# LPMP/BDD

Hardware: AMD Instinct MI355X
Metric: parallel-MMA iterations/sec, 10.5M BDD nodes, 1 GPU (+ achieved HBM GB/s in roofline) (higher is better)
Workload: dtype f32

## Files before the change

bdd_amd/capi.py:

```python
from __future__ import annotations

import ctypes as C
import os
import subprocess

_HERE = os.path.dirname(os.path.abspath(__file__))
LIB_PATH = os.path.abspath(os.environ["BDDMMA_LIB"]) if os.environ.get("BDDMMA_LIB") else os.path.join(_HERE, "csrc", "libbdd_mma_hip.so")

OK = 0
ERR_INVALID_ARGUMENT, ERR_INVALID_BDD, ERR_DEVICE, ERR_STATE, ERR_UNSUPPORTED, ERR_IO = -1, -2, -3, -4, -5, -6
F32, F64 = 0, 1
K_FORWARD_MM, K_BACKWARD_MM, K_FINISH_DELTA, K_OTHER, K_COUNT = 0, 1, 2, 3, 4


class Options(C.Structure):
    _fields_ = [("pack_width", C.c_uint32), ("wide_pack_width", C.c_uint32), ("deterministic", C.c_uint32),
                ("vars_per_bin", C.c_uint32), ("stage_cap", C.c_uint32), ("waves_per_block", C.c_uint32),
                ("keep_bdd_order", C.c_uint32), ("resident_sweeps", C.c_uint32), ("exchange_by_variable", C.c_uint32),
                ("variant_flags", C.c_uint32), ("pack_fill", C.c_uint32), ("pack_stagger", C.c_uint32)]


class LbfgsParams(C.Structure):
    _fields_ = [("history_size", C.c_int32), ("init_step_size", C.c_double), ("req_rel_lb_increase", C.c_double),
                ("step_size_decrease_factor", C.c_double), ("step_size_increase_factor", C.c_double)]


class LbfgsState(C.Structure):
    _fields_ = [("step_size", C.c_double), ("last_applied_step", C.c_double), ("mma_iterations", C.c_uint64),
                ("lbfgs_iterations", C.c_uint64), ("history_entries", C.c_int32), ("num_unsuccessful_updates", C.c_int32),
                ("last_kind", C.c_int32), ("last_trials", C.c_int32)]


class RunResult(C.Structure):
    _fields_ = [("iterations", C.c_uint64), ("lb_initial", C.c_double), ("lb_final", C.c_double),
                ("seconds", C.c_double), ("stop_reason", C.c_int32)]


class Profile(C.Structure):
    _fields_ = [("launches", C.c_uint64 * K_COUNT), ("total_ms", C.c_double * K_COUNT)]


_V, _U64, _I, _D = C.c_void_p, C.c_uint64, C.c_int, C.c_double
SIGNATURES = {
    "bddmma_create": (_I, [C.POINTER(_V), _I, _I, _V, _V, _U64, _V, _U64, C.POINTER(Options)]),
    "bddmma_destroy": (None, [_V]),
    "bddmma_device_count": (_I, []),
    "bddmma_device_chip": (_I, [_I, C.POINTER(C.c_uint32), C.POINTER(C.c_uint32), C.POINTER(C.c_uint64)]),
    "bddmma_set_layout_threads": (_I, [_I]),
    "bddmma_set_thread_layout_threads": (_I, [_I]),
    "bddmma_last_error": (C.c_char_p, [_V]),
    "bddmma_nr_variables": (_U64, [_V]),
    "bddmma_nr_bdds": (_U64, [_V]),
    "bddmma_nr_layers": (_U64, [_V]),
    "bddmma_nr_bdd_nodes": (_U64, [_V]),
    "bddmma_nr_hops": (_U64, [_V]),
    "bddmma_nr_packs": (_U64, [_V]),
    "bddmma_solve_sweep_kind": (_I, [_V]),
    "bddmma_fused_small": (_I, [_V]),
    "bddmma_fused_small_learned": (_I, [_V]),
    "bddmma_nontemporal_loads": (_I, [_V]),
    "bddmma_precision": (_I, [_V]),
    "bddmma_device": (_I, [_V]),
    "bddmma_num_bdds_per_var": (_I, [_V, _V]),
    "bddmma_layer_variables": (_I, [_V, _V]),
    "bddmma_layer_bdds": (_I, [_V, _V]),
    "bddmma_nodes_per_hop": (_I, [_V, _V]),
    "bddmma_layers_per_hop": (_I, [_V, _V]),
    "bddmma_update_costs": (_I, [_V, _V, _U64, _V, _U64, _I, _I]),
    "bddmma_set_cost": (_I, [_V, _D, _U64]),
    "bddmma_get_solver_costs": (_I, [_V, _V, _V, _V, _I]),
    "bddmma_set_solver_costs": (_I, [_V, _V, _V, _V, _I]),
    "bddmma_primal_objective_vec": (_I, [_V, _V, _I]),
    "bddmma_forward_run": (_I, [_V]),
    "bddmma_backward_run": (_I, [_V]),
    "bddmma_lower_bound": (_I, [_V, C.POINTER(_D)]),
    "bddmma_lower_bound_per_bdd": (_I, [_V, _V, _I]),
    "bddmma_iteration": (_I, [_V, _D]),
    "bddmma_iterations": (_I, [_V, _D, _U64]),
    "bddmma_learned_iterations": (_I, [_V, _V, _I, _U64, _D, _D, _V, _V, _V, _U64, _D, _I, C.POINTER(_U64)]),
    "bddmma_learned_iterations_omega_vec": (_I, [_V, _V, _I, _U64, _V, _I, _D, _V, _V, _V, _U64, _D, _I, C.POINTER(_U64)]),
    "bddmma_isotropic_dist_weights": (_I, [_V, _V, _I]),
    "bddmma_forward_mm": (_I, [_V, _D, _V, _I]),
    "bddmma_backward_mm": (_I, [_V, _D, _V, _I]),
    "bddmma_normalize_delta": (_I, [_V, _V, _I]),
    "bddmma_distribute_delta": (_I, [_V]),
    "bddmma_get_delta": (_I, [_V, _V, _I]),
    "bddmma_set_delta": (_I, [_V, _V, _I]),
    "bddmma_min_marginals": (_I, [_V, _I, _V, _V, _V, _I]),
    "bddmma_min_marginal_diff": (_I, [_V, _V, _I]),
    "bddmma_sum_marginals": (_I, [_V, _I, _I, _V, _V, _V, _I]),
    "bddmma_smooth_solution": (_I, [_V, _V, _I]),
    "bddmma_grad_min_marginal_diff": (_I, [_V, _V, _V, _V, _I]),
    "bddmma_grad_lower_bound_per_bdd": (_I, [_V, _V, _V, _V, _I, _I]),
    "bddmma_grad_distribute_delta": (_I, [_V, _V, _V, _V, _I]),
    "bddmma_grad_cost_perturbation": (_I, [_V, _V, _V, _V, _V, _I]),
    "bddmma_grad_learned_iterations": (_I, [_V, _V, _I, _D, _V, _I, _V, _V, _V, _V, _V, _U64, _U64, _U64, _I]),
    "bddmma_bdds_solution": (_I, [_V, _I, _V, _I]),
    "bddmma_net_solver_costs": (_I, [_V, _V, _I]),
    "bddmma_make_dual_feasible": (_I, [_V, _V, _I]),
    "bddmma_gradient_step": (_I, [_V, _V, _D, _I]),
    "bddmma_lbfgs_create": (_I, [C.POINTER(_V), _V, C.POINTER(LbfgsParams)]),
    "bddmma_lbfgs_destroy": (None, [_V]),
    "bddmma_lbfgs_iteration": (_I, [_V]),
    "bddmma_lbfgs_update_costs": (_I, [_V, _V, _U64, _V, _U64, _I, _I]),
    "bddmma_lbfgs_flush": (_I, [_V]),
    "bddmma_lbfgs_get_state": (_I, [_V, C.POINTER(LbfgsState)]),
    "bddmma_perturb_primal_costs": (_I, [_V, _V, _D, C.c_uint32, C.c_uint32, C.POINTER(C.c_uint32), _V, _V, _V]),
    "bddmma_run_solver": (_I, [_V, _V, _U64, _D, _D, _D, _I, C.POINTER(RunResult)]),
    "bddmma_run_solver_host_loop": (_I, [_V, _V, _U64, _D, _D, _D, _I, C.POINTER(RunResult)]),
    "bddmma_batch_create": (_I, [C.POINTER(_V), C.POINTER(_V), _U64]),
    "bddmma_batch_destroy": (None, [_V]),
    "bddmma_batch_last_error": (C.c_char_p, [_V]),
    "bddmma_batch_size": (_U64, [_V]),
    "bddmma_batch_iterations": (_I, [_V, _D, _U64]),
    "bddmma_learned_iterations_batch": (_I, [_V, _V, _V, _D, _U64, _I]),
    "bddmma_grad_learned_iterations_batch": (_I, [_V, _V, _V, _D, _V, _V, _V, _V, _V, _U64, _U64, _U64, _I]),
    "bddmma_set_solver_costs_batch": (_I, [_V, _V, _V, _V, _I]),
    "bddmma_get_solver_costs_batch": (_I, [_V, _V, _V, _V, _I]),
    "bddmma_stream_wait_batch": (_I, [_V, _V]),
    "bddmma_stream_signal_batch": (_I, [_V, _V]),
    "bddmma_batch_time_iterations": (_I, [_V, _D, _U64, C.POINTER(_D)]),
    "bddmma_batch_run_solver": (_I, [_V, _U64, _D, _D, _D, C.POINTER(RunResult)]),
    "bddmma_batch_lower_bounds": (_I, [_V, C.POINTER(_D)]),
    "bddmma_incremental_mm_agreement_rounding": (_I, [_V, _V, _D, _D, _U64, _U64, C.c_uint32, _I, _V, C.POINTER(_I)]),
    "bddmma_save": (_I, [_V, C.c_char_p]),
    "bddmma_load": (_I, [C.POINTER(_V), _I, C.c_char_p]),
    "bddmma_synchronize": (_I, [_V]),
    "bddmma_stream_wait": (_I, [_V, _V]),
    "bddmma_stream_signal": (_I, [_V, _V]),
    "bddmma_set_profiling": (_I, [_V, _I]),
    "bddmma_get_profile": (_I, [_V, C.POINTER(Profile)]),
    "bddmma_time_iterations": (_I, [_V, _D, _U64, C.POINTER(_D)]),
    "bddmma_time_kernel": (_I, [_V, _I, _U64, C.POINTER(_D)]),
    "bddmma_device_bytes": (_U64, [_V]),
    "bddmma_device_allocated_bytes": (_U64, [_V]),
    "bddmma_layout_create": (_I, [C.POINTER(_V), _V, _V, _U64, C.POINTER(Options)]),
    "bddmma_layout_create_for_chip": (_I, [C.POINTER(_V), _V, _V, _U64, C.POINTER(Options), _I, C.c_uint32, C.c_uint32]),
    "bddmma_layout_destroy": (None, [_V]),
    "bddmma_layout_size": (_U64, [_V, _I]),
    "bddmma_layout_copy": (_I, [_V, _I, _V]),
    "bddmma_layout_res2_records": (_I, [_V, _I, _V, _V, _V]),
    "bddmma_layout_stream_records": (_I, [_V, _I, _V, _V, _V]),
    "bddmma_layout_layer_records": (_I, [_V, _I, _V, _V, _V]),
# ... 68 lines not shown
```

bdd_amd/csrc/capi.cpp:

```cpp
#include <chrono>
#include <cmath>
#include <cstdio>
#include <cstdlib>
#include <cstring>
#include <limits>
#include <new>
#include <string>
#include <vector>

#include "../../include/bdd_mma.h"
#include "layout.hpp"
#include "solver.hpp"

using namespace bddmma;

struct bddmma_lbfgs;
extern "C" int bddmma_lbfgs_iteration(bddmma_lbfgs* l);
extern "C" int bddmma_lbfgs_update_costs(bddmma_lbfgs* l, const void* lo, uint64_t n_lo, const void* hi, uint64_t n_hi, int elem_precision,
                                         int on_device);

namespace {
thread_local std::string g_err;

template <typename F>
// ... 49 lines not shown
        constexpr bool timing = false;
#endif
        auto t_last = std::chrono::steady_clock::now();
        auto lap = [&](const char* what) {
            if (!timing) return;
            const auto now = std::chrono::steady_clock::now();
            std::fprintf(stderr, "[create] %-28s %8.1f ms\n", what, std::chrono::duration<double, std::milli>(now - t_last).count());
            t_last = now;
        };
        HostLayout L;
        ChipInfo chip;
        int rc = query_chip(device, &chip, g_err);
        if (rc) return rc;
        rc = build_layout(instr, bdd_delims, n_bdds, opts, L, g_err, false, precision == BDDMMA_F64 ? 8 : 4, chip);
        if (rc) return rc;
        lap("host layout");
        SolverBase* impl = nullptr;
        rc = create_solver(&impl, precision, device, L, opts, g_err);
        if (rc) return rc;
        lap("device buffers + upload");
        impl->n_packs_narrow = L.narrow.n_packs();
        impl->n_packs_wide = L.wide.n_packs() + L.huge.n_packs();
        if (costs_hi && n_costs) {
            rc = impl->update_costs(nullptr, 0, costs_hi, n_costs, BDDMMA_F64, 0);
            if (rc) {
                g_err = impl->err;
                delete impl;
                return rc;
            }
        }
        lap("update_costs");
        *out = new bddmma_solver{impl};
        return BDDMMA_OK;
    } catch (const std::exception& e) {
        g_err = e.what();
        return BDDMMA_ERR_DEVICE;
    }
}

int bddmma_device_count(void) { return device_count(); }
int bddmma_device_chip(int device, uint32_t* n_cus, uint32_t* lds_bytes_per_cu, uint64_t* max_resident_threads)
{
    if (device < 0 || device >= device_count()) { g_err = "no such HIP device"; return BDDMMA_ERR_DEVICE; }
    ChipInfo chip;
    const int rc = query_chip(device, &chip, g_err);
    if (rc) return rc;
    if (n_cus) *n_cus = chip.n_cus;
    if (lds_bytes_per_cu) *lds_bytes_per_cu = chip.lds_bytes;
    if (max_resident_threads) *max_resident_threads = chip.max_resident_threads;
    return BDDMMA_OK;
}
int bddmma_set_layout_threads(int n)
{
    if (n < 0) return BDDMMA_ERR_INVALID_ARGUMENT;
    set_layout_threads((unsigned)n);
    return BDDMMA_OK;
}
int bddmma_set_thread_layout_threads(int n)
{
    if (n < 0) return BDDMMA_ERR_INVALID_ARGUMENT;
    set_thread_layout_threads((unsigned)n);
    return BDDMMA_OK;
}

void bddmma_destroy(bddmma_solver* s)
{
    if (!s) return;
    delete s->impl;
    delete s;
}

const char* bddmma_last_error(const bddmma_solver* s) { return (s && s->impl) ? s->impl->err.c_str() : g_err.c_str(); }

uint64_t bddmma_nr_variables(const bddmma_solver* s) { return s && s->impl ? s->impl->n_vars : 0; }
uint64_t bddmma_nr_bdds(const bddmma_solver* s) { return s && s->impl ? s->impl->n_bdds : 0; }
uint64_t bddmma_nr_layers(const bddmma_solver* s) { return s && s->impl ? s->impl->n_layers : 0; }
uint64_t bddmma_nr_bdd_nodes(const bddmma_solver* s) { return s && s->impl ? s->impl->n_input_nodes : 0; }
uint64_t bddmma_nr_hops(const bddmma_solver* s) { return s && s->impl ? s->impl->n_hops : 0; }
uint64_t bddmma_nr_packs(const bddmma_solver* s) { return s && s->impl ? s->impl->n_packs_narrow + s->impl->n_packs_wide : 0; }
int bddmma_solve_sweep_kind(const bddmma_solver* s) { return s && s->impl ? s->impl->solve_sweep_kind : -1; }
int bddmma_fused_small(const bddmma_solver* s) { return s && s->impl ? (s->impl->fused_small ? 1 : 0) : -1; }
int bddmma_fused_small_learned(const bddmma_solver* s) { return s && s->impl ? (s->impl->fused_small_learned ? 1 : 0) : -1; }
int bddmma_nontemporal_loads(const bddmma_solver* s) { return s && s->impl ? (s->impl->nt_loads ? 1 : 0) : -1; }
int bddmma_precision(const bddmma_solver* s) { return s && s->impl ? s->impl->precision : -1; }
int bddmma_device(const bddmma_solver* s) { return s && s->impl ? s->impl->device : -1; }
uint64_t bddmma_device_bytes(const bddmma_solver* s) { return s && s->impl ? s->impl->dev_bytes : 0; }
uint64_t bddmma_device_allocated_bytes(const bddmma_solver* s) { return s && s->impl ? s->impl->dev_alloc_bytes : 0; }

int bddmma_num_bdds_per_var(const bddmma_solver* s, int32_t* out)
{
    return guarded(s, [&](SolverBase* b) { return copy_host(b->h_nbdds, out); });
}
int bddmma_layer_variables(const bddmma_solver* s, int32_t* out)
{
    return guarded(s, [&](SolverBase* b) { return copy_host(b->h_layer_var, out); });
}
int bddmma_layer_bdds(const bddmma_solver* s, int32_t* out)
{
    return guarded(s, [&](SolverBase* b) { return copy_host(b->h_layer_bdd, out); });
}
int bddmma_nodes_per_hop(const bddmma_solver* s, uint64_t* out)
{
    return guarded(s, [&](SolverBase* b) { return copy_host(b->nodes_per_hop, out); });
}
int bddmma_layers_per_hop(const bddmma_solver* s, uint64_t* out)
{
    return guarded(s, [&](SolverBase* b) { return copy_host(b->layers_per_hop, out); });
}

int bddmma_update_costs(bddmma_solver* s, const void* lo, uint64_t n_lo, const void* hi, uint64_t n_hi,
                        int elem_precision, int on_device)
{
    return guarded(s, [&](SolverBase* b) {
        if (elem_precision != BDDMMA_F32 && elem_precision != BDDMMA_F64) {
            b->err = "elem_precision must be BDDMMA_F32 or BDDMMA_F64";
            return BDDMMA_ERR_INVALID_ARGUMENT;
        }
        return b->update_costs(lo, n_lo, hi, n_hi, elem_precision, on_device);
    });
}
int bddmma_set_cost(bddmma_solver* s, double c, uint64_t var)
{
    return guarded(s, [&](SolverBase* b) { return b->set_cost(c, var); });
}
int bddmma_get_solver_costs(const bddmma_solver* s, void* lo, void* hi, void* mm, int on_device)
{
    return guarded(s, [&](SolverBase* b) { return b->get_solver_costs(lo, hi, mm, on_device); });
}
int bddmma_set_solver_costs(bddmma_solver* s, const void* lo, const void* hi, const void* mm, int on_device)
{
    return guarded(s, [&](SolverBase* b) { return b->set_solver_costs(lo, hi, mm, on_device); });
}
int bddmma_primal_objective_vec(bddmma_solver* s, void* out, int on_device)
{
    return guarded(s, [&](SolverBase* b) { return b->primal_objective_vec(out, on_device); });
}
int bddmma_forward_run(bddmma_solver* s) { return guarded(s, [&](SolverBase* b) { return b->forward_run(); }); }
int bddmma_backward_run(bddmma_solver* s) { return guarded(s, [&](SolverBase* b) { return b->backward_run(); }); }
int bddmma_lower_bound(bddmma_solver* s, double* lb)
{
    return guarded(s, [&](SolverBase* b) { return lb ? b->lower_bound(lb) : BDDMMA_ERR_INVALID_ARGUMENT; });
}
int bddmma_lower_bound_per_bdd(bddmma_solver* s, void* out, int on_device)
{
    return guarded(s, [&](SolverBase* b) { return b->lower_bound_per_bdd(out, on_device); });
}
int bddmma_iteration(bddmma_solver* s, double omega)
{
    return guarded(s, [&](SolverBase* b) { return b->iteration(omega); });
}
int bddmma_iterations(bddmma_solver* s, double omega, uint64_t n)
{
    return guarded(s, [&](SolverBase* b) { return b->iterations(omega, n); });
}
int bddmma_learned_iterations(bddmma_solver* s, const void* dist_weights, int weights_on_device, uint64_t num_itr, double omega,
                              double improvement_slope, void* sol_avg, void* lb_first_diff_avg, void* lb_second_diff_avg,
                              uint64_t compute_history_for_itr, double history_avg_beta, int outputs_on_device, uint64_t* itr_done)
{
    return guarded(s, [&](SolverBase* b) {
        return b->learned_iterations(dist_weights, weights_on_device, num_itr, omega, improvement_slope, sol_avg, lb_first_diff_avg,
                                     lb_second_diff_avg, compute_history_for_itr, history_avg_beta, outputs_on_device, itr_done, nullptr, 0);
    });
}
int bddmma_learned_iterations_omega_vec(bddmma_solver* s, const void* dist_weights, int weights_on_device, uint64_t num_itr, const void* omega_vec,
                                        int omega_vec_on_device, double improvement_slope, void* sol_avg, void* lb_first_diff_avg,
                                        void* lb_second_diff_avg, uint64_t compute_history_for_itr, double history_avg_beta, int outputs_on_device,
// ... 611 lines not shown
```

bdd_amd/csrc/kernels.hpp:

```cpp
#pragma once
#include <hip/hip_runtime.h>

#include <cstdint>
#include <type_traits>

#include "layout.hpp"

#include "kernels/common.hpp"
#include "kernels/stream.hpp"
#include "kernels/narrow.hpp"
#include "kernels/resident.hpp"
#include "kernels/narrow2.hpp"
#include "kernels/narrow3.hpp"
#include "kernels/wide.hpp"
#include "kernels/exchange.hpp"
#include "kernels/small.hpp"
#include "kernels/elementwise.hpp"
```

bdd_amd/csrc/solver.hpp:

```cpp
#pragma once
#include <hip/hip_runtime.h>

#include <cstdint>
#include <limits>
#include <memory>
#include <string>
#include <utility>
#include <vector>

#include "../../include/bdd_mma.h"
#include "layout.hpp"

namespace bddmma {

struct SolverBase {
    int precision = BDDMMA_F32, device = -1;
    hipStream_t stream = nullptr;
    std::string err;
    uint64_t n_vars = 0, n_bdds = 0, n_layers = 0, n_hops = 0, n_input_nodes = 0, n_slots = 0;
    int solve_sweep_kind = 0;
    uint32_t pack_width = 0, wide_pack_width = 0, wide_slot_base = 0;
    uint64_t dev_bytes = 0;
    uint64_t dev_alloc_bytes = 0;
    bool fwd_valid = false, bwd_valid = false;
    uint64_t cost_epoch = 0;
    bool deterministic = false;
    std::vector<uint64_t> nodes_per_hop, layers_per_hop;
    std::vector<int32_t> h_nbdds, h_layer_var, h_layer_bdd;
    std::vector<uint32_t> h_var_ptr;
    uint32_t n_packs_narrow = 0, n_packs_wide = 0;
    LayoutScalars lay_scalars{};
    bddmma_options saved_opts{};
    virtual int download_layout(HostLayout& H) = 0;
    virtual int init_from_layout(const HostLayout& L, const bddmma_options* opts) = 0;

    bool profiling = false;
    uint32_t prof_stride = 1;
    uint64_t prof_iter = 0;
    bool prof_active = false;
    std::vector<std::pair<hipEvent_t, hipEvent_t>> ev_pool;
    std::vector<int> ev_class;
    size_t ev_used = 0;
    hipEvent_t ev_t0 = nullptr, ev_t1 = nullptr;
    hipEvent_t ev_order = nullptr;

    virtual ~SolverBase() {}
    virtual int forward_run() = 0;
    virtual int backward_run() = 0;
    virtual int lower_bound(double* lb) = 0;
    virtual int lower_bound_enqueue(int slot) = 0;
    virtual int lower_bound_fetch(int slot, double* lb) = 0;
    virtual int lower_bound_per_bdd(void* out, int on_device) = 0;
    virtual int iteration(double omega) = 0;
    virtual int iterations(double omega, uint64_t n)
    {
        for (uint64_t i = 0; i < n; ++i)
            if (int rc = iteration(omega)) return rc;
        return BDDMMA_OK;
    }
    virtual int learned_iterations(const void* dist_weights, int weights_on_device, uint64_t num_itr, double omega, double improvement_slope,
                                   void* sol_avg, void* lb_first_diff_avg, void* lb_second_diff_avg, uint64_t compute_history_for_itr,
                                   double history_avg_beta, int outputs_on_device, uint64_t* itr_done, const void* omega_vec,
                                   int omega_vec_on_device) = 0;
    virtual int isotropic_dist_weights(void* out, int on_device) = 0;
    double initial_lb_change = std::numeric_limits<double>::infinity();
    std::shared_ptr<int> lbfgs_attached = std::make_shared<int>(0);
    bool fused_small = false;
    bool fused_small_learned = false;
    bool nt_loads = false;
    virtual int run_plain(uint64_t max_iter, double tolerance, double slope, double time_limit, int verbose, bddmma_run_result* res) = 0;
    virtual int forward_mm(double omega, void* delta, int on_device) = 0;
    virtual int backward_mm(double omega, void* delta, int on_device) = 0;
    virtual int normalize_delta(void* delta, int on_device) = 0;
    virtual int distribute_delta() = 0;
    virtual int get_delta(void* out, int on_device) = 0;
    virtual int set_delta(const void* in, int on_device) = 0;
    virtual int update_costs(const void* lo, uint64_t n_lo, const void* hi, uint64_t n_hi, int elem_precision, int on_device) = 0;
    virtual int set_cost(double c, uint64_t var) = 0;
    virtual int get_solver_costs(void* lo, void* hi, void* mm, int on_device) = 0;
    virtual int set_solver_costs(const void* lo, const void* hi, const void* mm, int on_device) = 0;
    virtual int primal_objective_vec(void* out, int on_device) = 0;
    virtual int min_marginals(int sorted, int32_t* var, void* mm0, void* mm1, int on_device) = 0;
    virtual int min_marginal_diff(void* out, int on_device) = 0;
    virtual int sum_marginals(int sorted, int log_probs, int32_t* var, void* sm0, void* sm1, int on_device) = 0;
    virtual int smooth_solution(void* out, int on_device) = 0;
    virtual int grad_min_marginal_diff(const void* grad_mm, void* grad_lo, void* grad_hi, int on_device) = 0;
    virtual int grad_lower_bound_per_bdd(const void* grad_lb, void* grad_lo, void* grad_hi, int smooth, int on_device) = 0;
    virtual int grad_distribute_delta(const void* grad_lo, const void* grad_hi, void* grad_deferred_mm, int on_device) = 0;
    virtual int grad_cost_perturbation(const void* grad_lo, const void* grad_hi, void* grad_lo_pert, void* grad_hi_pert, int on_device) = 0;
    virtual int grad_learned_iterations(const void* dist_weights, int weights_on_device, double omega, const void* omega_vec, int omega_vec_on_device,
                                        void* grad_lo, void* grad_hi, void* grad_mm, void* grad_dist_weights_out, void* grad_omega_out, uint64_t after,
                                        uint64_t n, uint64_t num_caches, int on_device) = 0;
    virtual int bdds_solution(int sorted, char* sol, int on_device) = 0;
    virtual int net_solver_costs(void* out, int on_device) = 0;
    virtual int make_dual_feasible(void* g, int on_device) = 0;
    virtual int gradient_step(const void* g, double step, int on_device) = 0;
    virtual int projection_means(const void* g_dev) = 0;
    virtual int gradient_step_projected(const void* g_dev, double step) = 0;
    virtual bool projection_fuses_lincomb() const = 0;
    virtual int projection_means_lincomb(const LinComb& lc, const void* tag) = 0;
    virtual void* stream_handle() = 0;
    struct LbfgsViews {
        const void* x_layer;
    };
    virtual int bdds_solution_async(char* dev_out, int prezeroed) = 0;
    virtual int lbfgs_views(LbfgsViews* out) = 0;
    virtual int time_kernel(int kind, uint64_t reps, double* ms) = 0;
    virtual int rounding_round(double delta, uint32_t round, uint32_t seed, uint32_t counts[4], char* sol_host, void* c0_host, void* c1_host,
                               bool apply_update, int* applied) = 0;
    virtual int rounding_scratch(void** c0_dev, void** c1_dev) = 0;

    int synchronize();
    int stream_wait(hipStream_t other);
    int stream_signal(hipStream_t other);
    void prof_begin(int kclass);
    void prof_end(int kclass);
    int set_profiling(int on);
    int get_profile(bddmma_profile* out);
    int time_iterations(double omega, uint64_t n, double* ms);
};

struct BatchBase {
    std::string err;
    virtual ~BatchBase() {}
    virtual uint64_t size() const = 0;
    virtual int iterations(double omega, uint64_t n) = 0;
    virtual int run_plain(uint64_t max_iter, double tolerance, double slope, double time_limit, bddmma_run_result* res) = 0;
    virtual int time_iterations(double omega, uint64_t n, double* ms) = 0;
    virtual int lower_bounds(double* out) = 0;
    virtual int learned_iterations(const void* dist_weights, const void* omega_vec, double omega, uint64_t num_itr, int on_device) = 0;
    virtual int grad_learned_iterations(const void* dist_weights, const void* omega_vec, double omega, void* grad_lo, void* grad_hi, void* grad_mm,
                                        void* grad_dist_weights_out, void* grad_omega_out, uint64_t track_grad_after_itr, uint64_t track_grad_for_num_itr,
                                        uint64_t num_caches, int on_device) = 0;
    virtual int set_solver_costs(const void* lo, const void* hi, const void* mm, int on_device) = 0;
    virtual int get_solver_costs(void* lo, void* hi, void* mm, int on_device) = 0;
    virtual int stream_wait(hipStream_t other) = 0;
    virtual int stream_signal(hipStream_t other) = 0;
};
int create_batch(BatchBase** out, SolverBase* const* members, uint64_t n, std::string& err);

int device_count();
int query_chip(int device, ChipInfo* out, std::string& err);
int create_solver(SolverBase** out, int precision, int device, const HostLayout& L, const bddmma_options* opts, std::string& err);

}

struct bddmma_solver {
    bddmma::SolverBase* impl = nullptr;
};
struct bddmma_batch {
    bddmma::BatchBase* impl = nullptr;
};
// ... 1 lines not shown
```

bdd_amd/csrc/solver_bt.hpp:

```cpp
#pragma once
#include <algorithm>
#include <mutex>

#include "solver_impl.hpp"
#include "kernels/gradsmall.hpp"
#include "kernels/batchcosts.hpp"

namespace bddmma {

template <typename REAL>
struct BatchT final : BatchBase {
    using S = SolverT<REAL>;
    using Fn = void (*)(const SmallItem<REAL>*, REAL, uint32_t);
    std::vector<S*> m;
    std::vector<uint32_t> order;
    struct Group {
        Fn fn;
        uint32_t threads, lds, first, count;
    };
    std::vector<Group> groups;
    int device = -1;
    hipStream_t stream = nullptr;
    std::vector<hipEvent_t> ev_in;
    hipEvent_t ev_out = nullptr, ev_chunk[2] = {nullptr, nullptr};
// ... 520 lines not shown
    {
        const uint32_t n = (uint32_t)m.size();
        if (!bc_ready) {
            std::vector<uint32_t> ord(n);
            for (uint32_t i = 0; i < n; ++i) ord[i] = i;
            std::stable_sort(ord.begin(), ord.end(), [&](uint32_t a, uint32_t b) { return m[a]->small_nw < m[b]->small_nw; });
            std::vector<uint64_t> src(n);
            uint64_t total = 0;
            for (uint32_t i = 0; i < n; ++i) {
                src[i] = total;
                total += m[i]->n_layers;
            }
            if (total > 0xFFFFFFFFull) { err = "batch solver costs: too many layers"; return BDDMMA_ERR_UNSUPPORTED; }
            std::vector<CostsItem<REAL>> items(n);
            std::vector<BcGroup> groups_;
            for (uint32_t j = 0; j < n; ++j) {
                const S* s = m[ord[j]];
                const SmallDev& sm = s->small;
                items[j] = CostsItem<REAL>{sm.pack_hdr, sm.rec, sm.rec_off, s->d_lpos, s->d_T, s->d_lohi, s->d_mm_binned, s->d_lb_partial,
                                           sm.rec_words, sm.ns, sm.nl, sm.n_packs, 0u, (uint32_t)s->n_layers, (uint32_t)src[ord[j]]};
                if (groups_.empty() || s->small_nw != m[ord[groups_.back().first]]->small_nw)
                    groups_.push_back(BcGroup{costs_set_fn<REAL>(s->small_nw), 64u * (uint32_t)s->small_nw, 0u, j, 0u});
                BcGroup& g = groups_.back();
                g.lds = std::max(g.lds, sm.n_packs * costs_region_bytes((uint32_t)sizeof(REAL), sm.ns, sm.nl));
                ++g.count;
            }
            for (const BcGroup& g : groups_) {
                if (g.lds > m[0]->lds_cu) { err = "batch set_solver_costs: the costs-to-terminal do not fit the LDS"; return BDDMMA_ERR_UNSUPPORTED; }
                if (int rc = raise_lds_limit(reinterpret_cast<const void*>(g.fn), g.lds)) return rc;
            }
            if (!d_bc_items) HIPCHK(hipMalloc((void**)&d_bc_items, n * sizeof(CostsItem<REAL>)));
            HIPCHK(hipMemcpy(d_bc_items, items.data(), n * sizeof(CostsItem<REAL>), hipMemcpyHostToDevice));
            bc_groups = std::move(groups_);
            bc_total = total;
            bc_ready = true;
        }
        if (host_arrays && bc_stage_cap < 3 * bc_total) {
            REAL* st = nullptr;
            HIPCHK(hipMalloc((void**)&st, std::max<uint64_t>(3 * bc_total, 1) * sizeof(REAL)));
            if (d_bc_stage) {
                (void)hipStreamSynchronize(stream);
                (void)hipFree(d_bc_stage);
            }
            d_bc_stage = st;
            bc_stage_cap = 3 * bc_total;
        }
        return BDDMMA_OK;
    }
    int members_in()
    {
        for (size_t i = 0; i < m.size(); ++i) {
            HIPCHK(hipEventRecord(ev_in[i], m[i]->stream));
            HIPCHK(hipStreamWaitEvent(stream, ev_in[i], 0));
        }
        return BDDMMA_OK;
    }
    int set_solver_costs(const void* lo, const void* hi, const void* mm, int on_dev) override
    {
        int rc;
        if ((rc = check_state())) return rc;
        if (!lo && !hi && !mm) return BDDMMA_OK;
        HIPCHK(hipSetDevice(device));
        if ((rc = bc_prepare(!on_dev))) return rc;
        if ((rc = members_in())) return rc;
        const REAL* a[3] = {(const REAL*)lo, (const REAL*)hi, (const REAL*)mm};
        hipError_t e = hipSuccess;
        if (!on_dev)
            for (int k = 0; k < 3 && e == hipSuccess; ++k)
                if (a[k]) {
                    REAL* const st = d_bc_stage + (uint64_t)k * bc_total;
                    e = hipMemcpyAsync(st, a[k], bc_total * sizeof(REAL), hipMemcpyHostToDevice, stream);
                    a[k] = st;
                }
        for (size_t g = 0; g < bc_groups.size() && e == hipSuccess; ++g) {
            const BcGroup& G = bc_groups[g];
            hipLaunchKernelGGL(G.fn, dim3(G.count), dim3(G.threads), G.lds, stream, (const CostsItem<REAL>*)(d_bc_items + G.first), a[0], a[1], a[2]);
            e = hipGetLastError();
        }
        if (e == hipSuccess && !on_dev) e = hipStreamSynchronize(stream);
        for (S* s : m) {
            s->costs_changed();
            s->lb_cached = false;
            ++s->lb_gen;
            s->bwd_valid = e == hipSuccess;
        }
        const int rc2 = join_out();
        if (e != hipSuccess) { err = std::string("batch set_solver_costs: ") + hipGetErrorString(e); return BDDMMA_ERR_DEVICE; }
        return rc2;
    }
    int get_solver_costs(void* lo, void* hi, void* mm, int on_dev) override
    {
        int rc;
        if ((rc = check_state())) return rc;
        if (!lo && !hi && !mm) return BDDMMA_OK;
        HIPCHK(hipSetDevice(device));
        if ((rc = bc_prepare(!on_dev))) return rc;
        if ((rc = members_in())) return rc;
        void* const out[3] = {lo, hi, mm};
        REAL* o[3];
        for (int k = 0; k < 3; ++k) o[k] = !out[k] ? nullptr : on_dev ? (REAL*)out[k] : d_bc_stage + (uint64_t)k * bc_total;
        hipLaunchKernelGGL(costs_get_fn<REAL>(), dim3((uint32_t)m.size()), dim3(256), 0, stream, (const CostsItem<REAL>*)d_bc_items, o[0], o[1], o[2]);
        hipError_t e = hipGetLastError();
        if (!on_dev) {
            for (int k = 0; k < 3 && e == hipSuccess; ++k)
                if (out[k]) e = hipMemcpyAsync(out[k], o[k], bc_total * sizeof(REAL), hipMemcpyDeviceToHost, stream);
            if (e == hipSuccess) e = hipStreamSynchronize(stream);
        }
        const int rc2 = join_out();
        if (e != hipSuccess) { err = std::string("batch get_solver_costs: ") + hipGetErrorString(e); return BDDMMA_ERR_DEVICE; }
        return rc2;
    }
    int stream_wait(hipStream_t other) override
    {
        HIPCHK(hipSetDevice(device));
        if (!ev_order) HIPCHK(hipEventCreateWithFlags(&ev_order, hipEventDisableTiming));
        HIPCHK(hipEventRecord(ev_order, other));
        HIPCHK(hipStreamWaitEvent(stream, ev_order, 0));
        return BDDMMA_OK;
    }
    int stream_signal(hipStream_t other) override
    {
        HIPCHK(hipSetDevice(device));
        if (!ev_order) HIPCHK(hipEventCreateWithFlags(&ev_order, hipEventDisableTiming));
        HIPCHK(hipEventRecord(ev_order, stream));
        HIPCHK(hipStreamWaitEvent(other, ev_order, 0));
        return BDDMMA_OK;
    }

    int lower_bounds(double* out) override
    {
        HIPCHK(hipSetDevice(device));
        std::vector<char> pending(m.size(), 0);
        for (size_t i = 0; i < m.size(); ++i) {
            S* s = m[i];
            int rc = s->backward_run();
            if (!rc && !s->lb_cached) {
                rc = s->launch_bound(0);
                pending[i] = 1;
            }
            if (rc) { err = s->err; return rc; }
        }
        for (size_t i = 0; i < m.size(); ++i) {
            S* s = m[i];
            if (pending[i]) {
                if (int rc = s->wait_bound(0)) { err = s->err; return rc; }
                s->lb_cache = ((volatile double*)s->h_lb)[0];
                s->lb_cached = true;
            }
            out[i] = s->lb_cache;
        }
        return BDDMMA_OK;
    }

    int run_plain(uint64_t max_iter, double tolerance, double slope, double time_limit, bddmma_run_result* res) override
    {
        if (slope < 0.0 || slope >= 1.0 || time_limit < 0.0 || tolerance < 0.0) {
            err = "run_solver: invalid termination criteria";
            return BDDMMA_ERR_INVALID_ARGUMENT;
        }
        int rc;
        if ((rc = check_state())) return rc;
        HIPCHK(hipSetDevice(device));
        const auto t0 = std::chrono::steady_clock::now();
        auto elapsed = [&]() { return std::chrono::duration<double>(std::chrono::steady_clock::now() - t0).count(); };
        const uint32_t n = (uint32_t)m.size();
        std::vector<double> lb_initial(n);
        if ((rc = lower_bounds(lb_initial.data()))) return rc;
// ... 81 lines not shown
```

bdd_amd/csrc/solver_impl.hpp:

```cpp
#pragma once
#include <hip/hip_runtime.h>
#include <atomic>
#include <chrono>
#include <cmath>
#include <cstdio>
#include <cstdlib>
#include <cstring>
#include <limits>
#include <memory>
#include <string>
#include <thread>
#include <type_traits>
#include <vector>
#include "../../include/bdd_mma.h"
#include "kernels.hpp"
#include "layout.hpp"
#include "solver.hpp"

namespace bddmma {

static inline void cpu_relax()
{
#if defined(__x86_64__) || defined(__i386__)
    __asm__ __volatile__("pause");
// ... 12 lines not shown
            err = std::string(#expr) + ": " + hipGetErrorString(e_);                                   \
            return BDDMMA_ERR_DEVICE;                                                                  \
        }                                                                                              \
    } while (0)

static inline uint32_t cdiv(uint64_t a, uint32_t b) { return (uint32_t)((a + b - 1) / b); }

template <int V0, int... Vs, class F>
decltype(auto) pick(uint32_t v, F&& f)
{
    if constexpr (sizeof...(Vs) == 0) return f(std::integral_constant<int, V0>{});
    else return v == (uint32_t)V0 ? f(std::integral_constant<int, V0>{}) : pick<Vs...>(v, static_cast<F&&>(f));
}

template <typename REAL, typename... TAIL>
struct PullSweep {
    using Fn = void (*)(DevPtrs<REAL>, PackDev, const uint32_t*, const uint32_t*, uint32_t, unsigned char*, TAIL...);
    Fn narrow, wide, huge;
    size_t (*bytes)(size_t, uint32_t);
    unsigned char* scratch;
};

#ifndef BDDMMA_EX_ACC
#define BDDMMA_EX_ACC double
#endif
template <typename REAL> struct GradSmallItem;
template <typename REAL> struct GradSmallIO;
template <typename REAL>
struct SolverT final : SolverBase {
    uint32_t* d_nwords = nullptr;
    uint32_t* d_pack_word_off = nullptr;
    uint32_t n_nwords = 0;
    uint64_t* d_wwords = nullptr;
    REAL *d_F = nullptr, *d_T = nullptr, *d_lohi = nullptr;
    REAL* d_lo = nullptr;
    REAL* d_hi = nullptr;
    int32_t *d_var = nullptr, *d_bdd = nullptr, *d_nbdds = nullptr;
    uint32_t *d_var_ptr = nullptr, *d_var_layers = nullptr, *d_root_slot = nullptr;
    REAL* d_delta_var = nullptr;
    bool delta_var_valid = true;
    REAL* d_delta_lay = nullptr;
    REAL* d_mm_binned = nullptr;
    REAL *d_delta_c = nullptr, *d_delta_lay_c = nullptr;
    REAL* d_alpha_ent = nullptr;
    REAL* d_omega_lay = nullptr;
    REAL* d_hist = nullptr;
    REAL* d_hist_out = nullptr;
    uint16_t* d_bvar = nullptr;
    uint32_t *d_evar = nullptr, *d_lpos = nullptr, *d_vpos = nullptr, *d_bin_ptr = nullptr;
    uint32_t *d_pack_group_ptr = nullptr, *d_grp_layer_off = nullptr, *d_grp_hop_end = nullptr;
    uint32_t *d_quad_round_ptr = nullptr, *d_cs_ptr = nullptr, *d_cs_entry = nullptr;
    uint16_t* d_cs_slot = nullptr;
    uint32_t wpb = 1;
    bool entry_by_var = false;
    bool exch_small = false, exch_medium = false;
    bool use_seg = false;
    uint32_t *d_seg_bin = nullptr, *d_seg_thr = nullptr;
    uint16_t* d_seg_perm = nullptr;
    uint32_t seg_lds = 0, seg_tile_off = 0, seg_cnt_off = 0, seg_groups = 0;
    bool big = false;
    uint32_t opts_variant = 0;
    uint32_t n_cus = 256, lds_cu = 160 * 1024;
    bool narrow_seg = false;
    uint32_t vars_per_bin = 0, n_bins = 0, stage_cap = 0, stage_lds = 0, exch_lds = 0, n_narrow_layers = 0;
    double *d_lb_partial = nullptr, *d_lb = nullptr;
    double* h_lb = nullptr;
    uint64_t *h_lb_seq = nullptr, *d_lb_seq = nullptr;
    uint64_t lb_seq_next = 0, lb_seq_expect[3] = {0, 0, 0};
    bool lb_cached = false;
    double lb_cache = 0.0;
    bool lb_slot_known[2] = {false, false}, lb_slot_enqueued[2] = {false, false};
    double lb_slot_value[2] = {0.0, 0.0};
    uint64_t lb_gen = 0, lb_slot_gen[2] = {0, 0};
    RunCtl* d_run_ctl = nullptr;
    RunHost *h_run = nullptr, *d_run_host = nullptr;
    const uint32_t* run_stop = nullptr;
    uint32_t run_iter = 0;
    RunGate gate() const { return RunGate{run_stop, run_iter}; }
    RunStep run_step{};
    REAL* d_x_layer = nullptr;
    bool x_layer_valid = false;
    void costs_changed()
    {
        fwd_valid = bwd_valid = x_layer_valid = false;
        ++cost_epoch;
    }
    CostQuot* d_cost_q = nullptr;
    uint8_t* d_cost_flags = nullptr;
    uint32_t* d_counts = nullptr;
    REAL *d_tmp0 = nullptr, *d_tmp1 = nullptr;
    char* d_sol = nullptr;
    struct PackBufs {
        uint32_t *pack_hop_ptr = nullptr, *hop_node_off = nullptr, *hop_layer_off = nullptr;
        uint8_t* pack_steps = nullptr;
        uint16_t* hop_root = nullptr;
        uint32_t n_packs = 0;
    } nb_, wb_, hb_;
    uint32_t wide_lds = 0, wide_threads = 256, wide_npt = 1;
    bool n3_nt = false;
    bool beyond_cache = false;
    bool n12_nt = false;
    uint32_t nt_potentials = 0;
    bool mixed = false;
    bool mixed_fwd = true;
    uint32_t mixed_npt = 1, mixed_lds = 0;
    uint32_t *d_pack_hdr = nullptr, *d_quad_hdr = nullptr;
    bool use_res = false;
    uint32_t res_ns = 0, res_nl = 0, res_lds = 0;
    bool use_res2 = false;
    uint32_t *d_res2_rec = nullptr, *d_res2_rec_off = nullptr;
    uint32_t res2_n_words = 0, res2_lds = 0, res2_ns = 0, res2_nl = 0;
    bool use_narrow2 = false, narrow_gen = false;
    uint32_t *d_srec = nullptr, *d_srec_off = nullptr;
    bool res_hdr_ok = false;
    const uint32_t* n2_hdr_pack() const { return res_hdr_ok ? d_pack_hdr : nullptr; }
    const uint32_t* n2_hdr_quad() const { return res_hdr_ok ? d_quad_hdr : nullptr; }
    uint32_t srec_words = 0;
    bool small_ok = false, small_rl = false;
    int small_nw = 1;
    uint32_t small_lds = 0;
    SmallDev small{};
    uint32_t* d_small_lds = nullptr;
    bool small_ln_ok = false, small_ln_rl = false, sl_ready = false;
    uint32_t small_ln_lds = 0;
    SmallDev small_ln{};
    SmallLearn<REAL> small_ln_arg{};
    bool use_narrow3 = false;
    uint32_t *d_lrec = nullptr, *d_lrec_off = nullptr;
    uint32_t lrec_words = 0;
    uint32_t huge_pack_width = 0;
    unsigned char* d_huge_scratch = nullptr;

    std::vector<void*> allocs;

    ~SolverT() override
    {
        if (device >= 0) (void)hipSetDevice(device);
        for (void* p : allocs) (void)hipFree(p);
        if (h_lb) (void)hipHostFree(h_lb);
        if (h_lb_seq) (void)hipHostFree(h_lb_seq);
        if (h_run) (void)hipHostFree(h_run);
        if (d_run_ctl) (void)hipFree(d_run_ctl);
        for (auto& e : ev_pool) {
            (void)hipEventDestroy(e.first);
            (void)hipEventDestroy(e.second);
        }
        if (ev_t0) (void)hipEventDestroy(ev_t0);
        if (ev_t1) (void)hipEventDestroy(ev_t1);
        if (ev_order) (void)hipEventDestroy(ev_order);
        if (stream) (void)hipStreamDestroy(stream);
    }

    struct Arena { char* base = nullptr; uint64_t size = 0, used = 0; };
    std::vector<Arena> arenas;
    uint64_t arena_chunk = 0;
    uint64_t arena_skew = 0;
    template <typename T>
    int dalloc(T** p, uint64_t n)
    {
        const uint64_t bytes = std::max<uint64_t>(n, 1) * sizeof(T) + 1024;
        if (arena_chunk == 0) {
            HIPCHK(hipMalloc((void**)p, bytes));
            allocs.push_back(*p);
            dev_bytes += bytes;
            dev_alloc_bytes += bytes;
            return BDDMMA_OK;
        }
        const uint64_t need = (bytes + 4095) / 4096 * 4096 + arena_skew;
        if (arenas.empty() || arenas.back().used + need > arenas.back().size) {
            Arena a;
            a.size = std::max(arenas.empty() ? arena_chunk : std::min<uint64_t>(arena_chunk, 64ull << 20), need);
            HIPCHK(hipMalloc((void**)&a.base, a.size));
            allocs.push_back(a.base);
            arenas.push_back(a);
            dev_alloc_bytes += a.size;
        }
        Arena& a = arenas.back();
        *p = reinterpret_cast<T*>(a.base + a.used);
        a.used += need;
        dev_bytes += bytes;
        return BDDMMA_OK;
    }
    struct DevField { const void* ptr = nullptr; uint64_t count = 0; };
    DevField dev_fields[LAYOUT_ARRAY_IDS];
    template <typename T>
    int upload(T** p, const std::vector<T>& h, int id = 0)
    {
        int rc = dalloc(p, h.size());
        if (rc) return rc;
        if (!h.empty()) HIPCHK(hipMemcpyAsync(*p, h.data(), h.size() * sizeof(T), hipMemcpyHostToDevice, stream));
        if (id) dev_fields[id] = DevField{*p, h.size()};
        return BDDMMA_OK;
    }
    int download_layout(HostLayout& H) override
    {
        HIPCHK(hipSetDevice(device));
        H = HostLayout();
        set_layout_scalars(H, lay_scalars);
        hipError_t e = hipSuccess;
        visit_layout_arrays(H, [&](int id, auto& vec) {
            using T = typename std::remove_reference_t<decltype(vec)>::value_type;
            if (id == LAY_NODES_PER_HOP) { vec.assign(nodes_per_hop.begin(), nodes_per_hop.end()); return; }
            if (id == LAY_LAYERS_PER_HOP) { vec.assign(layers_per_hop.begin(), layers_per_hop.end()); return; }
            const DevField& f = dev_fields[id];
            vec.resize(f.count);
            if (f.count && e == hipSuccess) e = hipMemcpyAsync(vec.data(), f.ptr, f.count * sizeof(T), hipMemcpyDeviceToHost, stream);
        });
        if (e == hipSuccess) e = hipStreamSynchronize(stream);
        HIPCHK(e);
        return BDDMMA_OK;
// ... 162 lines not shown
                seg_cnt_off = seg_tile_off + SE.max_slots * 2u * (uint32_t)sizeof(REAL);
                seg_lds = (seg_cnt_off + SE.max_slots * 2u + 15u) & ~15u;
                if (seg_lds + 1024 <= lds_cu) {
                    if ((rc = upload(&d_seg_bin, SE.bin))) return rc;
                    if ((rc = upload(&d_seg_perm, SE.perm))) return rc;
                    if ((rc = upload(&d_seg_thr, SE.thr))) return rc;
                    use_seg = true;
                    seg_groups = SE.max_groups;
                }
            }
        }
        if ((rc = upload(&d_pack_hdr, L.res.pack_hdr, LAY_PACK_HDR))) return rc;
        if ((rc = upload(&d_quad_hdr, L.res.quad_hdr, LAY_QUAD_HDR))) return rc;
        res_hdr_ok = L.res.ok && nb_.n_packs > 0;
        if (nb_.n_packs && L.res.ok) {
            res_ns = (L.res.max_slots + 255) / 256 * 256;
            res_nl = (L.res.max_layers + 127) / 128 * 128;
            res_lds = wpb * stage_cap * 2 * (uint32_t)sizeof(REAL) + wpb * res_wave_bytes(sizeof(REAL), res_ns, res_nl);
            const uint32_t static_lds = wpb * (2 * (pack_width + 2) * (uint32_t)sizeof(REAL) + 512) + seg_bytes(wpb);
            const uint32_t mode = opts ? opts->resident_sweeps : 0;
            const bool fits = res_lds + static_lds <= lds_cu - 512;
            const uint64_t wgs_per_cu = fits ? (lds_cu) / (res_lds + static_lds) : 0;
            const bool all_in_flight = (uint64_t)nb_.n_packs * 256 <= 2880ull * n_cus && (uint64_t)cdiv(nb_.n_packs, wpb) <= (uint64_t)n_cus * std::min<uint64_t>(wgs_per_cu, 2048 / (64 * wpb));
            use_res = fits && mode != 1 && (mode == 2 || all_in_flight) && !big;
            if (pack_width == 64 && !narrow_seg && mode != 1 && !big && !(opts && (opts->variant_flags & 0x800u))) {
                res2_ns = res2_slot_capacity((uint32_t)sizeof(REAL), L.res.max_slots);
                res2_nl = res2_layer_capacity((uint32_t)sizeof(REAL), L.res.max_layers);
                res2_lds = wpb * stage_cap * 2 * (uint32_t)sizeof(REAL) + wpb * res2_wave_bytes(sizeof(REAL), res2_ns, res2_nl);
                const uint64_t wgs2 = res2_lds + 256 <= lds_cu ? std::min<uint64_t>((lds_cu) / (res2_lds + 256), 2048 / (64 * wpb)) : 0;
                const uint64_t in_flight = (uint64_t)n_cus * wgs2 * wpb;
                const bool auto_ok = sizeof(REAL) == 4 ? (uint64_t)nb_.n_packs * 100 <= in_flight * 145 : (uint64_t)nb_.n_packs <= in_flight;
                if (wgs2 && (mode == 2 || auto_ok)) {
                    Res2Records R2;
                    build_res2_records(L, sizeof(REAL), res2_ns, res2_nl, R2);
                    if (R2.ok && R2.rec.size() * sizeof(uint32_t) < (1ull << 31)) {
                        if ((rc = upload(&d_res2_rec, R2.rec))) return rc;
                        if ((rc = upload(&d_res2_rec_off, R2.rec_off))) return rc;
                        res2_n_words = (uint32_t)R2.rec.size();
                        use_res2 = use_res = true;
                    }
                }
            }
        }
        uint32_t narrow2_static = 0;
        if (nb_.n_packs && !use_res && !wb_.n_packs && !(opts && (opts->variant_flags & 0x1000u))) {
            StreamRecords SR;
            build_stream_records(L, sizeof(REAL), SR);
            narrow2_static = L.ex.waves_per_block * ((2 * pack_width + 2 + pack_width + 2) * (uint32_t)sizeof(REAL) + 3 * 64 * 4 + 64);
            const bool forced = opts && (opts->variant_flags & 0x2000u);
            const bool shared = forced || (SR.rec.size() * sizeof(uint32_t) <= (uint64_t)L.narrow_slots * sizeof(REAL) / 2 &&
                                           (sizeof(REAL) == 8 || n_slots <= 16'000'000ull));
            if (SR.ok && shared && stage_lds + narrow2_static + seg_bytes(L.ex.waves_per_block) <= 64 * 1024) {
                if ((rc = upload(&d_srec, SR.rec))) return rc;
                if ((rc = upload(&d_srec_off, SR.rec_off))) return rc;
                srec_words = (uint32_t)SR.rec.size();
                use_narrow2 = true;
                narrow_gen = narrow_seg;
                for (uint16_t r : L.narrow.hop_root) narrow_gen = narrow_gen || r != NO_ROOT;
            }
        }
        if (nb_.n_packs && !use_res && !wb_.n_packs && !hb_.n_packs && !narrow_seg && pack_width == 128 && (L.ex.waves_per_block == 4 || L.ex.waves_per_block == 8) &&
            !(opts && (opts->variant_flags & 0x41000u))) {
            LayerRecords LR;
            build_layer_records(L, sizeof(REAL), LR);
            const uint32_t n3_static = L.ex.waves_per_block * (4 * (128 + 128) * (uint32_t)sizeof(REAL) + 3 * 64 * 4);
            const bool forced = opts && (opts->variant_flags & 0x2000u);
            const bool shared = forced || (LR.rec.size() * sizeof(uint32_t) <= (uint64_t)L.narrow_slots * sizeof(REAL) / 2 && n_slots <= 16'000'000ull);
            if (LR.ok && shared && stage_lds + n3_static <= lds_cu - 1024) {
                if ((rc = upload(&d_lrec, LR.rec))) return rc;
                if ((rc = upload(&d_lrec_off, LR.rec_off))) return rc;
                lrec_words = (uint32_t)LR.rec.size();
                use_narrow3 = true;
                n3_nt = sizeof(REAL) == 8 && nt_potentials != 0;
            }
        }
        if (nb_.n_packs && !use_res && !use_narrow3 && !wb_.n_packs && !hb_.n_packs && !narrow_seg && !narrow_gen && pack_width == 128 &&
            (L.ex.waves_per_block == 4 || L.ex.waves_per_block == 8) && (beyond_cache || (opts && (opts->variant_flags & 0x100000u))))
#ifndef BDDMMA_EXP_NO_N12_NT
            n12_nt = !use_narrow2 || sizeof(REAL) == 8;
#else
            n12_nt = false;
#endif
        nt_loads = n3_nt || n12_nt;
        if (wb_.n_packs) {
            wide_threads = std::min<uint32_t>(1024, std::max<uint32_t>(64, ((wide_pack_width + 1) / 2 + 63) / 64 * 64));
            wide_npt = (wide_pack_width + wide_threads - 1) / wide_threads;
            wide_npt = wide_npt <= 1 ? 1 : (wide_npt <= 2 ? 2 : 4);
            wide_lds = (uint32_t)wide2_lds_bytes(sizeof(REAL), wide_pack_width, true);
            if (wide_lds > lds_cu || wide_pack_width > 4096) {
                err = "wide_pack_width " + std::to_string(wide_pack_width) + " needs " + std::to_string(wide_lds) + " B of LDS (> 160 KiB)";
                return BDDMMA_ERR_UNSUPPORTED;
            }
        }
        if (wb_.n_packs && nb_.n_packs && !use_res && !(opts && (opts->variant_flags & 1u))) {
            const uint32_t threads = 64 * wpb;
            const uint32_t npt = (wide_pack_width + threads - 1) / threads;
            const uint32_t narrow_dyn = stage_lds + seg_bytes(wpb);
            if (npt <= 4 && wide_lds <= narrow_dyn + 16 * 1024 && std::max(narrow_dyn, wide_lds) + narrow_static <= 64 * 1024) {
                mixed = true;
                mixed_npt = npt <= 1 ? 1 : (npt <= 2 ? 2 : 4);
                mixed_lds = std::max(narrow_dyn, wide_lds);
            }
        }
        if (use_res2 && res_hdr_ok && nb_.n_packs <= SMALL_MAX_PACKS && !wb_.n_packs && !hb_.n_packs && !deterministic && !entry_by_var && !big &&
            L.var_ptr.size() == n_vars + 1 && L.ex.vpos.size() == n_layers && !(opts && (opts->variant_flags & 0x80000u))) {
            const uint32_t np = nb_.n_packs;
            std::vector<uint32_t> lds_off(n_layers);
            uint32_t max_hops = 0;
            bool ok = true;
            for (uint32_t k = 0; k < (uint32_t)n_layers && ok; ++k) {
                const uint32_t l = L.var_layers[k];
                uint32_t p = 0;
                while (p < np && !(l >= L.res.pack_hdr[8 * (size_t)p + 2] && l < L.res.pack_hdr[8 * (size_t)p + 2] + L.res.pack_hdr[8 * (size_t)p + 3])) ++p;
                if (p == np || l - L.res.pack_hdr[8 * (size_t)p + 2] >= res2_nl) { ok = false; break; }
                lds_off[k] = (p * small_stage_stride(res2_nl) + (l - L.res.pack_hdr[8 * (size_t)p + 2])) * 2u * (uint32_t)sizeof(REAL);
            }
            for (uint32_t p = 0; p < np; ++p) max_hops = std::max(max_hops, L.res.pack_hdr[8 * (size_t)p + 5] & 0xFFFFu);
            small = SmallDev{};
            small.ns = res2_ns; small.nl = res2_nl; small.n_packs = np; small.wpb = wpb; small.n_quads = cdiv(np, wpb);
            small.n_vars = (uint32_t)n_vars; small.n_entries = (uint32_t)n_layers; small.rec_words = res2_n_words;
            small.rec_cap = (max_hops + 1u) * 1024u;
            uint32_t bytes = small_lds_bytes((uint32_t)sizeof(REAL), np, (uint32_t)n_vars, (uint32_t)n_layers, small);
            small_rl = bytes + 512 <= lds_cu;
            if (!small_rl) {
                small.rec_cap = 0;
                bytes = small_lds_bytes((uint32_t)sizeof(REAL), np, (uint32_t)n_vars, (uint32_t)n_layers, small);
            }
            if (ok && bytes + 512 <= lds_cu) {
                if ((rc = upload(&d_small_lds, lds_off))) return rc;
                small.pack_hdr = d_pack_hdr; small.quad_hdr = d_quad_hdr; small.rec = d_res2_rec; small.rec_off = d_res2_rec_off;
                small.var_ptr = d_var_ptr; small.var_lds = d_small_lds; small.var_ent = d_vpos;
                small_lds = bytes;
                small_nw = np <= 1 ? 1 : np <= 2 ? 2 : np <= 4 ? 4 : np <= 8 ? 8 : 16;
                small_ok = true;
                fused_small = true;
                small_ln = small;
                small_ln.rec_cap = (max_hops + 1u) * 1024u;
                uint32_t max_layers = 0;
                for (uint32_t p = 0; p < np; ++p) max_layers = std::max(max_layers, L.res.pack_hdr[8 * (size_t)p + 3]);
                small_ln_arg.om_stride = max_layers;
                auto learned_bytes = [&]() {
                    const uint32_t plain = small_lds_bytes((uint32_t)sizeof(REAL), np, (uint32_t)n_vars, (uint32_t)n_layers, small_ln);
                    return small_learn_lds_bytes((uint32_t)sizeof(REAL), np, res2_nl, max_layers, plain, small_ln_arg.off_om);
                };
                uint32_t lbytes = learned_bytes();
                small_ln_rl = lbytes + 512 <= lds_cu;
                if (!small_ln_rl) {
                    small_ln.rec_cap = 0;
                    lbytes = learned_bytes();
                }
                if (lbytes + 512 <= lds_cu) {
                    small_ln_lds = lbytes;
                    small_ln_ok = true;
                    fused_small_learned = true;
                }
            }
        }
        resolve_kernels();
        if ((rc = raise_lds_limits(kern))) return rc;
        solve_sweep_kind = !nb_.n_packs ? BDDMMA_SWEEPS_NONE : mixed ? BDDMMA_SWEEPS_MIXED : (use_res && use_res2) ? BDDMMA_SWEEPS_RESIDENT2 : use_res ? BDDMMA_SWEEPS_RESIDENT1
                           : use_narrow3 ? BDDMMA_SWEEPS_STREAMING3 : use_narrow2 ? BDDMMA_SWEEPS_STREAMING2 : BDDMMA_SWEEPS_STREAMING1;
        HIPCHK(hipStreamSynchronize(stream));
        return BDDMMA_OK;
    }

    DevPtrs<REAL> ptrs(const REAL* delta_lay) const
    {
        DevPtrs<REAL> d;
        d.nwords = d_nwords; d.n_nwords = n_nwords; d.wwords = d_wwords; d.wide_slot_base = wide_slot_base;
        d.F = d_F; d.T = d_T; d.lohi = d_lohi;
        d.delta_lay = delta_lay; d.mm_binned = d_mm_binned; d.lpos = d_lpos; d.cs_entry = d_cs_entry; d.cs_slot = d_cs_slot;
        d.n_slots = (uint32_t)n_slots; d.n_layers = (uint32_t)n_layers; d.n_narrow_layers = n_narrow_layers;
        d.lb_partial = d_lb_partial;
        d.mm0_out = d_tmp0; d.mm1_out = d_tmp1; d.sol_out = d_sol;
        d.x_layer = d_x_layer;
        d.stop = run_stop;
        d.run_iter = run_iter;
        d.big = big ? 1u : 0u;
        return d;
    }
    PackDev pdev(const PackBufs& b, uint32_t lb_base, uint32_t seg_off = 0) const
    {
        const bool narrow_set = &b == &nb_;
        return PackDev{b.pack_hop_ptr, b.hop_node_off, b.hop_layer_off, b.pack_steps, b.hop_root, d_pack_word_off,
                       d_pack_group_ptr, d_grp_layer_off, d_grp_hop_end, d_quad_round_ptr, d_cs_ptr, stage_cap, seg_off, b.n_packs, lb_base,
                       nt_potentials, xcd_chunk(), narrow_set ? n2_hdr_pack() : nullptr, narrow_set ? n2_hdr_quad() : nullptr};
    }
    uint32_t seg_bytes(uint32_t w) const { return narrow_seg ? w * 128 * (uint32_t)sizeof(REAL) : 0; }
    uint32_t xcd_chunk_auto = 0;
    uint32_t xcd_chunk() const { return xcd_chunk_auto; }
    uint32_t narrow_grid(uint32_t n_quads) const
    {
        const uint32_t c = xcd_chunk();
        return c ? 8 * c * cdiv(n_quads, 8 * c) : 8 * cdiv(n_quads, 8);
    }

    template <typename FN>
    struct Kern { FN fn = nullptr; uint32_t lds = 0; };
    using NarrowFn = void (*)(DevPtrs<REAL>, PackDev, REAL);
    using RecFn = void (*)(DevPtrs<REAL>, PackDev, const uint32_t*, const uint32_t*, uint32_t, REAL);
    using ResFn = void (*)(const uint32_t*, const uint32_t*, uint32_t, uint32_t, uint32_t, uint32_t, const uint32_t*, uint32_t, DevPtrs<REAL>, PackDev, REAL);
    using Res2Fn = void (*)(const uint32_t*, const uint32_t*, uint32_t, uint32_t, uint32_t, uint32_t, const uint32_t*, uint32_t, const uint32_t*,
                            const uint32_t*, uint32_t, DevPtrs<REAL>, PackDev, REAL);
    using WideFn = void (*)(DevPtrs<REAL>, PackDev, REAL, uint32_t);
    using HugeFn = void (*)(DevPtrs<REAL>, PackDev, REAL, uint32_t, unsigned char*);
    using MixedFn = void (*)(DevPtrs<REAL>, PackDev, PackDev, REAL, uint32_t);
    using ExFn = void (*)(const REAL*, const uint32_t*, const uint16_t*, const uint32_t*, uint32_t, uint32_t, uint32_t, uint32_t, const int32_t*, REAL*, REAL*,
                          RunStep, const REAL*);
    using SegFn = void (*)(const REAL*, const uint4*, const uint32_t*, uint32_t, const uint4*, const uint2*, uint32_t, uint32_t, REAL*, RunStep, const REAL*);
    using ProjFn = void (*)(REAL*, const uint32_t*, const uint16_t*, const int32_t*, uint32_t, uint32_t, uint32_t);
    using SmallFn = void (*)(SmallDev, DevPtrs<REAL>, PackDev, REAL, uint32_t, RunStep);
    using TransFn = void (*)(const REAL*, REAL*, PackDev, const uint32_t*, const uint16_t*, uint32_t, uint32_t, REAL*, REAL);
    using LincombFn = void (*)(LinComb, REAL*, PackDev, const uint32_t*, const uint16_t*, uint32_t, uint32_t);
    struct Sweep {
        Res2Fn res2 = nullptr;
        ResFn res = nullptr;
        RecFn rec = nullptr;
        NarrowFn narrow = nullptr;
        uint32_t narrow_lds = 0, w = 1, seg_off = 0;
        const uint32_t *rec_tab = nullptr, *rec_off = nullptr;
        uint32_t rec_words = 0;
        Kern<WideFn> wide;
        Kern<MixedFn> mixed;
        HugeFn huge = nullptr;
        const void* narrow_fn() const { return res2 ? (const void*)res2 : res ? (const void*)res : rec ? (const void*)rec : (const void*)narrow; }
    };
    struct Kernels {
        Sweep sweep[2][3];
        uint32_t ex_threads = 0;
        Kern<ExFn> ex[2], ex_w, ex_raw;
        Kern<SegFn> seg[2], seg_w;
        Kern<ProjFn> project;
        Kern<SmallFn> small;
        Kern<TransFn> transpose[2];
        Kern<LincombFn> lincomb[2];
    } kern;
    Sweep ov_sweep[2];
    template <int MODE, bool OV>
    Sweep resolve_sweep(bool bwd) const
    {
        constexpr bool SOLVE = MODE == FWD_SOLVE;
        static_assert(!OV || SOLVE, "omega per layer: solve sweeps only");
        Sweep s;
        if (hb_.n_packs) s.huge = bwd ? &k_bwd_wide<REAL, MODE, true, OV> : &k_fwd_wide<REAL, MODE, true, OV>;
        if (wb_.n_packs)
            s.wide = {pick<1, 2, 4>(wide_npt, [&](auto N) -> WideFn { return bwd ? &k_bwd_wide2<REAL, MODE, N.value, OV> : &k_fwd_wide2<REAL, MODE, N.value, OV>; }),
                      wide_lds};
        if (!nb_.n_packs) return s;
        if constexpr (!SOLVE) {
            s.narrow = pick<64, 128, 256>(pack_width, [&](auto PW) -> NarrowFn {
                constexpr int R = PW.value / 64;
                return bwd ? &k_bwd_narrow<REAL, R, MODE, 1, true, false, false> : &k_fwd_narrow<REAL, R, MODE, 1, true, false, false>;
            });
            s.narrow_lds = seg_bytes(1);
        } else {
            s.w = wpb;
            s.seg_off = use_res ? res_lds : stage_lds;
            s.narrow_lds = (use_res && use_res2) ? res2_lds : s.seg_off + seg_bytes(wpb);
            pick<64, 128, 256>(pack_width, [&](auto PW) {
                pick<1, 2, 4, 8>(wpb, [&](auto W_) {
                    constexpr int R = PW.value / 64, W = W_.value, W48 = W == 8 ? 8 : 4;
                    const bool w48 = W == 4 || W == 8;
                    if (use_res && use_res2) s.res2 = bwd ? &k_bwd_res2<REAL, W, OV> : &k_fwd_res2<REAL, W, OV>;
                    else if (use_res) s.res = bwd ? &k_bwd_res<REAL, R, W, OV> : &k_fwd_res<REAL, R, W, OV>;
                    else if (use_narrow3 && w48) {
                        s.rec = bwd ? &k_bwd_narrow3<REAL, W48, false, OV> : &k_fwd_narrow3<REAL, W48, false, OV>;
                        if constexpr (sizeof(REAL) == 8)
                            if (n3_nt) s.rec = bwd ? &k_bwd_narrow3<REAL, W48, true, OV> : &k_fwd_narrow3<REAL, W48, true, OV>;
                        s.rec_tab = d_lrec; s.rec_off = d_lrec_off; s.rec_words = lrec_words;
                    } else if (use_narrow2) {
                        if (n12_nt && R == 2 && w48) s.rec = bwd ? &k_bwd_narrow2<REAL, 2, W48, false, sizeof(REAL) == 8, OV> : &k_fwd_narrow2<REAL, 2, W48, false, sizeof(REAL) == 8, OV>;
                        else if (narrow_gen) s.rec = bwd ? &k_bwd_narrow2<REAL, R, W, true, false, OV> : &k_fwd_narrow2<REAL, R, W, true, false, OV>;
                        else s.rec = bwd ? &k_bwd_narrow2<REAL, R, W, false, false, OV> : &k_fwd_narrow2<REAL, R, W, false, false, OV>;
                        s.rec_tab = d_srec; s.rec_off = d_srec_off; s.rec_words = srec_words;
                    } else if (n12_nt && R == 2 && w48) s.narrow = bwd ? &k_bwd_narrow<REAL, 2, MODE, W48, false, true, OV> : &k_fwd_narrow<REAL, 2, MODE, W48, false, true, OV>;
                    else if (!narrow_seg) s.narrow = bwd ? &k_bwd_narrow<REAL, R, MODE, W, false, false, OV> : &k_fwd_narrow<REAL, R, MODE, W, false, false, OV>;
                    else s.narrow = bwd ? &k_bwd_narrow<REAL, R, MODE, W, true, false, OV> : &k_fwd_narrow<REAL, R, MODE, W, true, false, OV>;
                });
            });
            if (mixed)
                s.mixed = {pick<64, 128, 256>(pack_width, [&](auto PW) {
                               return pick<1, 2, 4, 8>(wpb, [&](auto W) {
                                   return pick<1, 2, 4>(mixed_npt, [&](auto N) -> MixedFn {
                                       constexpr int R = PW.value / 64;
                                       return bwd ? &k_bwd_mixed<REAL, R, W.value, N.value, OV> : &k_fwd_mixed<REAL, R, W.value, N.value, OV>;
                                   });
                               });
                           }),
                           mixed_lds};
        }
        return s;
    }
    void resolve_kernels()
    {
        for (int bwd = 0; bwd < 2; ++bwd) {
            kern.sweep[bwd][FWD_PLAIN] = resolve_sweep<FWD_PLAIN, false>(bwd);
            kern.sweep[bwd][FWD_SOLVE] = resolve_sweep<FWD_SOLVE, false>(bwd);
            kern.sweep[bwd][FWD_SOLUTION] = resolve_sweep<FWD_SOLUTION, false>(bwd);
        }
        kern.ex_threads = exch_small ? EXS_THREADS : exch_medium ? EXM_THREADS : EX_THREADS;
        pick<EXS_THREADS, EXM_THREADS, EX_THREADS>(kern.ex_threads, [&](auto T_) {
            constexpr int T = T_.value, U = T == EXS_THREADS ? EXS_UNROLL : T == EXM_THREADS ? EXM_UNROLL : EX_UNROLL,
                          N = T == EXS_THREADS ? EXS_NPT : T == EXM_THREADS ? EXM_NPT : EX_NPT;
            kern.ex[0] = {&k_exchange_reduce<REAL, BDDMMA_EX_ACC, EX_ITER, T, U, N, false>, exch_lds};
            kern.ex[1] = {&k_exchange_reduce<REAL, BDDMMA_EX_ACC, EX_ITER, T, U, N, true>, exch_lds};
            kern.ex_w = {&k_exchange_reduce<REAL, BDDMMA_EX_ACC, EX_ITER, T, U, N, false, true>, exch_lds};
            kern.project = {&k_project_entries<REAL, T>, vars_per_bin * (uint32_t)sizeof(double)};
            if (use_seg)
                pick<2, 4>(seg_groups <= 2 ? 2 : 4, [&](auto G) {
                    kern.seg[0] = {&k_exchange_seg<REAL, T, G.value, false>, seg_lds};
                    kern.seg[1] = {&k_exchange_seg<REAL, T, G.value, true>, seg_lds};
                    kern.seg_w = {&k_exchange_seg<REAL, T, G.value, false, true>, seg_lds};
                });
        });
        kern.ex_raw = {&k_exchange_reduce<REAL, BDDMMA_EX_ACC, EX_RAW>, exch_lds};
        if (small_ok)
            kern.small = {pick<1, 2, 4, 8, 16>(small_nw, [&](auto NW) -> SmallFn {
                              return small_rl ? &k_iterate_small<REAL, NW.value, true> : &k_iterate_small<REAL, NW.value, false>;
                          }),
                          small_lds};
        if (n_narrow_layers)
            pick<1, 2, 4, 8>(wpb, [&](auto W) {
                const uint32_t lds = wpb * stage_cap * (uint32_t)sizeof(REAL);
                kern.transpose[0] = {&k_stage_transpose<REAL, W.value, 0>, lds};
                kern.transpose[1] = {&k_stage_transpose<REAL, W.value, 1>, lds};
                kern.lincomb[0] = {&k_stage_lincomb<REAL, W.value, 0>, lds};
                kern.lincomb[1] = {&k_stage_lincomb<REAL, W.value, 5>, lds};
            });
    }
    int raise_lds_limit(const void* fn, uint32_t lds)
    {
        if (fn && lds) HIPCHK(hipFuncSetAttribute(fn, hipFuncAttributeMaxDynamicSharedMemorySize, (int)lds));
        return BDDMMA_OK;
    }
    template <typename FN>
    int raise_lds_limit(const Kern<FN>& k) { return raise_lds_limit(reinterpret_cast<const void*>(k.fn), k.lds); }
    int raise_lds_limits(const Sweep& s)
    {
        if (int rc = raise_lds_limit(s.narrow_fn(), s.narrow_lds)) return rc;
        return raise_lds_limit(s.wide);
    }
    int raise_lds_limits(const Kernels& k)
    {
        int rc = BDDMMA_OK;
        for (const auto& dir : k.sweep)
            for (const Sweep& s : dir)
                if ((rc = raise_lds_limits(s))) return rc;
        for (const auto* e : {&k.ex[0], &k.ex[1], &k.ex_w, &k.ex_raw})
            if ((rc = raise_lds_limit(*e))) return rc;
        for (const auto* e : {&k.seg[0], &k.seg[1], &k.seg_w})
            if ((rc = raise_lds_limit(*e))) return rc;
        for (const auto* e : {&k.transpose[0], &k.transpose[1]})
            if ((rc = raise_lds_limit(*e))) return rc;
        for (const auto* e : {&k.lincomb[0], &k.lincomb[1]})
            if ((rc = raise_lds_limit(*e))) return rc;
        if ((rc = raise_lds_limit(k.project))) return rc;
        return raise_lds_limit(k.small);
    }

    int ov_prepare();
    using SmallLnFn = void (*)(SmallDev, DevPtrs<REAL>, PackDev, SmallLearn<REAL>, REAL, uint32_t);
    using SmallLnBatchFn = void (*)(const SmallLearnItem<REAL>*, REAL, uint32_t, uint32_t);
    Kern<SmallLnFn> small_ln_kern;
    int sl_prepare();
    static SmallLnBatchFn sl_batch_fn(int nw, bool rl);
    using GradSmallFn = void (*)(const GradSmallItem<REAL>*, REAL, uint32_t, uint32_t, GradSmallIO<REAL>);
    using GradSmallLoadFn = void (*)(const GradSmallItem<REAL>*, GradSmallIO<REAL>, uint32_t*);
    static GradSmallFn gs_batch_fn(int nw, bool rl);
    static GradSmallLoadFn gs_load_fn();
    bool ov_ready = false;
    int launch_sweep(bool bwd, const Sweep& s, const REAL* delta_lay, REAL omega, int kclass, bool ov = false)
    {
        if (bwd) {
            lb_cached = false;
            ++lb_gen;
        }
        DevPtrs<REAL> d = ptrs(delta_lay);
        if (ov) d.omega_lay = d_omega_lay;
        prof_begin(kclass);
        if (s.mixed.fn && (bwd || mixed_fwd)) {
            const PackDev pkw = pdev(wb_, nb_.n_packs), pkn = pdev(nb_, 0, stage_lds);
            const uint32_t nw8 = (wb_.n_packs + 7u) & ~7u;
            const dim3 grid(nw8 + narrow_grid(cdiv(nb_.n_packs, wpb))), block(64 * wpb);
            hipLaunchKernelGGL(s.mixed.fn, grid, block, s.mixed.lds, stream, d, pkn, pkw, omega, wide_pack_width);
        } else {
            if (s.wide.fn) hipLaunchKernelGGL(s.wide.fn, dim3(wb_.n_packs), dim3(wide_threads), s.wide.lds, stream, d, pdev(wb_, nb_.n_packs), omega, wide_pack_width);
            if (nb_.n_packs) {
                const PackDev pk = pdev(nb_, 0, s.seg_off);
                const dim3 grid(narrow_grid(cdiv(nb_.n_packs, s.w))), block(64 * s.w);
                if (s.res2)
                    hipLaunchKernelGGL(s.res2, grid, block, s.narrow_lds, stream, d_pack_hdr, d_quad_hdr, res2_ns, res2_nl, pk.n_packs, pk.xcd_chunk, d.stop, d.run_iter,
                                       d_res2_rec, d_res2_rec_off, res2_n_words, d, pk, omega);
                else if (s.res)
                    hipLaunchKernelGGL(s.res, grid, block, s.narrow_lds, stream, d_pack_hdr, d_quad_hdr, res_ns, res_nl, pk.n_packs, pk.xcd_chunk, d.stop, d.run_iter, d, pk, omega);
                else if (s.rec) hipLaunchKernelGGL(s.rec, grid, block, s.narrow_lds, stream, d, pk, s.rec_tab, s.rec_off, s.rec_words, omega);
                else hipLaunchKernelGGL(s.narrow, grid, block, s.narrow_lds, stream, d, pk, omega);
            }
        }
        if (s.huge) hipLaunchKernelGGL(s.huge, dim3(hb_.n_packs), dim3(WIDE_THREADS), 0, stream, d, pdev(hb_, nb_.n_packs + wb_.n_packs), omega, huge_pack_width, d_huge_scratch);
        prof_end(kclass);
        HIPCHK(hipGetLastError());
        return BDDMMA_OK;
    }
    int launch_fwd(int mode, const REAL* delta_lay, REAL omega, int kclass) { return launch_sweep(false, kern.sweep[0][mode], delta_lay, omega, kclass); }
    int launch_bwd(int mode, const REAL* delta_lay, REAL omega, int kclass) { return launch_sweep(true, kern.sweep[1][mode], delta_lay, omega, kclass); }
    void launch_bcast(const REAL* delta_var, REAL* delta_lay, RunGate g = RunGate{}, RunStep run = RunStep{})
    {
        hipLaunchKernelGGL((k_exchange_bcast<REAL>), dim3(cdiv(cdiv(n_layers, 4), 256)), dim3(256), 0, stream, delta_var, d_evar, delta_lay,
                           (uint32_t)n_layers, (uint32_t)n_vars, g, run);
    }
    void launch_reduce_raw(REAL* delta_var)
    {
        if (deterministic)
            hipLaunchKernelGGL((k_delta_gather<REAL, false>), dim3(cdiv(n_vars, 256)), dim3(256), 0, stream, d_mm_binned, d_var_ptr,
                               d_vpos, delta_var, (uint32_t)n_vars, RunGate{});
        else
            hipLaunchKernelGGL(kern.ex_raw.fn, dim3(n_bins), dim3(EX_THREADS), kern.ex_raw.lds, stream, d_mm_binned, d_bin_ptr, d_bvar,
                               (const uint32_t*)nullptr, 0u, vars_per_bin, (uint32_t)n_vars, (uint32_t)n_layers, d_nbdds, delta_var, (REAL*)nullptr, RunStep{},
                               (const REAL*)nullptr);
    }
    int exchange(bool ends_iteration = false)
    {
        const RunStep rstep = (ends_iteration && run_stop) ? run_step : RunStep{};
        prof_begin(BDDMMA_K_FINISH_DELTA);
        if (entry_by_var) {
            hipLaunchKernelGGL((k_exchange_byvar<REAL>), dim3(cdiv(n_vars, 256)), dim3(256), 0, stream, d_mm_binned, d_var_ptr, d_delta_lay,
                               (uint32_t)n_vars, (uint32_t)n_layers, gate(), rstep);
            delta_var_valid = false;
        } else if (deterministic && !use_seg) {
            hipLaunchKernelGGL((k_delta_gather<REAL, true>), dim3(cdiv(n_vars, 256)), dim3(256), 0, stream, d_mm_binned, d_var_ptr,
                               d_vpos, d_delta_var, (uint32_t)n_vars, gate());
            launch_bcast(d_delta_var, d_delta_lay, gate(), rstep);
            delta_var_valid = true;
        } else {
            const bool run = run_stop != nullptr;
            const dim3 grid(n_bins + (run && rstep.ctl != nullptr ? 1u : 0u)), block(kern.ex_threads);
            if (use_seg)
                hipLaunchKernelGGL(kern.seg[run].fn, grid, block, kern.seg[run].lds, stream, d_mm_binned, reinterpret_cast<const uint4*>(d_seg_bin), gate().stop,
                                   gate().iter, reinterpret_cast<const uint4*>(d_seg_perm), reinterpret_cast<const uint2*>(d_seg_thr), seg_tile_off, seg_cnt_off,
                                   d_delta_lay, rstep, (const REAL*)nullptr);
            else
                hipLaunchKernelGGL(kern.ex[run].fn, grid, block, kern.ex[run].lds, stream, d_mm_binned, d_bin_ptr, d_bvar, gate().stop, gate().iter, vars_per_bin,
                                   (uint32_t)n_vars, (uint32_t)n_layers, d_nbdds, (REAL*)nullptr, d_delta_lay, rstep, (const REAL*)nullptr);
            delta_var_valid = false;
        }
        prof_end(BDDMMA_K_FINISH_DELTA);
        HIPCHK(hipGetLastError());
        return BDDMMA_OK;
    }

    int forward_run() override
    {
        if (fwd_valid) return BDDMMA_OK;
        HIPCHK(hipSetDevice(device));
        int rc = launch_fwd(FWD_PLAIN, nullptr, REAL(0), BDDMMA_K_OTHER);
        if (rc) return rc;
        fwd_valid = true;
        return BDDMMA_OK;
    }
    int backward_run() override
    {
        if (bwd_valid) return BDDMMA_OK;
        HIPCHK(hipSetDevice(device));
        int rc = launch_bwd(BWD_PLAIN, nullptr, REAL(0), BDDMMA_K_OTHER);
        if (rc) return rc;
        bwd_valid = true;
        return BDDMMA_OK;
    }
    int lower_bound(double* lb) override
    {
        int rc = backward_run();
        if (rc) return rc;
        if (lb_cached) {
            *lb = lb_cache;
            return BDDMMA_OK;
        }
        if ((rc = launch_bound(0))) return rc;
        if ((rc = wait_bound(0))) return rc;
        *lb = lb_cache = ((volatile double*)h_lb)[0];
        lb_cached = true;
        return BDDMMA_OK;
    }
    int launch_bound(int k)
    {
        lb_seq_expect[k] = ++lb_seq_next;
        hipLaunchKernelGGL(k_lb_reduce, dim3(1), dim3(1024), 0, stream, d_lb_partial, nb_.n_packs + wb_.n_packs + hb_.n_packs, d_lb + k, d_lb_seq + k, lb_seq_expect[k]);
        HIPCHK(hipGetLastError());
        return BDDMMA_OK;
    }
    int wait_bound(int k)
    {
        volatile uint64_t* w = h_lb_seq + k;
        const auto t0 = std::chrono::steady_clock::now();
        uint32_t spins = 0;
        while (*w != lb_seq_expect[k]) {
            cpu_relax();
            if ((++spins & 1023u) == 0 && std::chrono::duration<double>(std::chrono::steady_clock::now() - t0).count() > 2e-3) {
                HIPCHK(hipStreamSynchronize(stream));
                if (*w != lb_seq_expect[k]) { err = "lower bound: the reduce kernel did not report"; return BDDMMA_ERR_DEVICE; }
                break;
            }
        }
        std::atomic_thread_fence(std::memory_order_acquire);
        return BDDMMA_OK;
    }
    int lower_bound_enqueue(int slot) override
    {
        if (slot < 0 || slot > 1) { err = "lower_bound_enqueue: slot must be 0 or 1"; return BDDMMA_ERR_INVALID_ARGUMENT; }
        int rc = backward_run();
        if (rc) return rc;
        lb_slot_gen[slot] = lb_gen;
        if (lb_cached) {
            lb_slot_known[slot] = true;
            lb_slot_value[slot] = lb_cache;
            return BDDMMA_OK;
        }
        if ((rc = launch_bound(1 + slot))) return rc;
        lb_slot_known[slot] = false;
        lb_slot_enqueued[slot] = true;
        return BDDMMA_OK;
    }
    int lower_bound_fetch(int slot, double* lb) override
    {
        if (slot < 0 || slot > 1) { err = "lower_bound_fetch: slot must be 0 or 1"; return BDDMMA_ERR_INVALID_ARGUMENT; }
        if (!lb_slot_known[slot]) {
            if (!lb_slot_enqueued[slot]) { err = "lower_bound_fetch without lower_bound_enqueue"; return BDDMMA_ERR_STATE; }
            int rc = wait_bound(1 + slot);
            if (rc) return rc;
            lb_slot_value[slot] = ((volatile double*)h_lb)[1 + slot];
            lb_slot_known[slot] = true;
        }
        *lb = lb_slot_value[slot];
        if (lb_slot_gen[slot] == lb_gen && bwd_valid) {
            lb_cache = *lb;
            lb_cached = true;
        }
        return BDDMMA_OK;
    }
    int lower_bound_per_bdd(void* out, int on_device) override
    {
        int rc = backward_run();
        if (rc) return rc;
        REAL* tmp = nullptr;
        REAL* dst = (REAL*)out;
        if (!on_device) { HIPCHK(hipMalloc((void**)&tmp, n_bdds * sizeof(REAL))); dst = tmp; }
        hipLaunchKernelGGL((k_lb_per_bdd<REAL>), dim3(cdiv(n_bdds, 256)), dim3(256), 0, stream, d_T, d_root_slot, dst, (uint32_t)n_bdds);
        if (!on_device) {
            hipError_t e = hipMemcpyAsync(out, tmp, n_bdds * sizeof(REAL), hipMemcpyDeviceToHost, stream);
            if (e == hipSuccess) e = hipStreamSynchronize(stream);
            (void)hipFree(tmp);
            HIPCHK(e);
        }
        return BDDMMA_OK;
    }

    int mma_forward(REAL omega, const REAL* delta_lay, bool ov = false)
    {
        int rc;
        if (!bwd_valid && (rc = backward_run())) return rc;
        rc = launch_sweep(false, ov ? ov_sweep[0] : kern.sweep[0][FWD_SOLVE], delta_lay, omega, BDDMMA_K_FORWARD_MM, ov);
        x_layer_valid = false;
        if (rc) return rc;
        fwd_valid = true;
        bwd_valid = false;
        return BDDMMA_OK;
    }
    int mma_backward(REAL omega, const REAL* delta_lay, bool ov = false)
    {
        if (!fwd_valid) {
            err = "backward_mm requires a valid forward state (call forward_mm first)";
            return BDDMMA_ERR_STATE;
        }
        int rc = launch_sweep(true, ov ? ov_sweep[1] : kern.sweep[1][BWD_SOLVE], delta_lay, omega, BDDMMA_K_BACKWARD_MM, ov);
        if (rc) return rc;
        x_layer_valid = d_x_layer != nullptr;
        fwd_valid = false;
        bwd_valid = true;
        return BDDMMA_OK;
    }
    bool small_usable() const { return small_ok && !profiling && d_x_layer == nullptr; }
    void small_launched()
    {
        lb_cached = false;
        ++lb_gen;
        x_layer_valid = false;
        fwd_valid = false;
        bwd_valid = true;
        delta_var_valid = false;
    }
    int launch_small(REAL omega, uint32_t n, const RunStep& rstep)
    {
        int rc;
        if (!bwd_valid && (rc = backward_run())) return rc;
        const DevPtrs<REAL> d = ptrs(d_delta_lay);
        const PackDev pk = pdev(nb_, 0, 0);
        hipLaunchKernelGGL(kern.small.fn, dim3(1), dim3(64 * small_nw), kern.small.lds, stream, small, d, pk, omega, n, rstep);
        HIPCHK(hipGetLastError());
        small_launched();
        return BDDMMA_OK;
    }
    bool small_learned_usable() const { return small_ln_ok && small_usable(); }
    int launch_small_learned(REAL omega, bool ov, uint32_t n)
    {
        int rc;
        if (!sl_ready) {
            if ((rc = sl_prepare())) return rc;
            sl_ready = true;
        }
        if (!bwd_valid && (rc = backward_run())) return rc;
        SmallLearn<REAL> ln = small_ln_arg;
        ln.alpha_ent = d_alpha_ent;
        ln.omega_lay = ov ? d_omega_lay : nullptr;
        hipLaunchKernelGGL(small_ln_kern.fn, dim3(1), dim3(64 * small_nw), small_ln_kern.lds, stream, small_ln, ptrs(d_delta_lay), pdev(nb_, 0, 0), ln, omega, n);
        HIPCHK(hipGetLastError());
        small_launched();
        return BDDMMA_OK;
    }
    SmallLearnItem<REAL> small_learn_item() const
    {
        SmallLearn<REAL> ln = small_ln_arg;
        ln.alpha_ent = d_alpha_ent;
        ln.omega_lay = d_omega_lay;
        return SmallLearnItem<REAL>{small_ln, ptrs(d_delta_lay), pdev(nb_, 0, 0), ln};
    }
    SmallItem<REAL> small_item() const { return SmallItem<REAL>{small, ptrs(d_delta_lay), pdev(nb_, 0, 0), RunStep{d_lb_partial, nb_.n_packs + wb_.n_packs + hb_.n_packs, nullptr, nullptr}}; }
    int iterations(double omega, uint64_t n) override
    {
        HIPCHK(hipSetDevice(device));
        if (!small_usable() || run_stop) {
            for (uint64_t i = 0; i < n; ++i)
                if (int rc = iteration(omega)) return rc;
            return BDDMMA_OK;
        }
        while (n) {
            const uint32_t chunk = (uint32_t)std::min<uint64_t>(n, 1u << 14);
            if (int rc = launch_small((REAL)omega, chunk, RunStep{})) return rc;
            n -= chunk;
        }
        return BDDMMA_OK;
    }
    int iteration(double omega) override
    {
        HIPCHK(hipSetDevice(device));
        int rc;
        if (small_usable() && !run_stop) return launch_small((REAL)omega, 1, RunStep{});
        prof_active = profiling && (prof_iter++ % prof_stride == 0);
        if ((rc = mma_forward((REAL)omega, d_delta_lay))) return rc;
        if ((rc = exchange())) return rc;
        if ((rc = mma_backward((REAL)omega, d_delta_lay))) return rc;
        if ((rc = exchange(true))) return rc;
        return BDDMMA_OK;
    }
    void weighted_exchange()
    {
        const REAL* al = d_alpha_ent;
        prof_begin(BDDMMA_K_FINISH_DELTA);
        if (entry_by_var) {
            hipLaunchKernelGGL((k_exchange_byvar<REAL, true>), dim3(cdiv(n_vars, 256)), dim3(256), 0, stream, d_mm_binned, d_var_ptr, d_delta_lay,
                               (uint32_t)n_vars, (uint32_t)n_layers, RunGate{}, RunStep{}, al);
        } else if (deterministic && !use_seg) {
            hipLaunchKernelGGL((k_delta_gather<REAL, false>), dim3(cdiv(n_vars, 256)), dim3(256), 0, stream, d_mm_binned, d_var_ptr,
                               d_vpos, d_delta_c, (uint32_t)n_vars, RunGate{});
            hipLaunchKernelGGL((k_exchange_bcast<REAL, true>), dim3(cdiv(cdiv(n_layers, 4), 256)), dim3(256), 0, stream, (const REAL*)d_delta_c, d_evar,
                               d_delta_lay, (uint32_t)n_layers, (uint32_t)n_vars, RunGate{}, RunStep{}, al);
        } else if (use_seg) {
            hipLaunchKernelGGL(kern.seg_w.fn, dim3(n_bins), dim3(kern.ex_threads), kern.seg_w.lds, stream, d_mm_binned, reinterpret_cast<const uint4*>(d_seg_bin),
                               (const uint32_t*)nullptr, 0u, reinterpret_cast<const uint4*>(d_seg_perm), reinterpret_cast<const uint2*>(d_seg_thr), seg_tile_off,
                               seg_cnt_off, d_delta_lay, RunStep{}, al);
        } else {
            hipLaunchKernelGGL(kern.ex_w.fn, dim3(n_bins), dim3(kern.ex_threads), kern.ex_w.lds, stream, d_mm_binned, d_bin_ptr, d_bvar, (const uint32_t*)nullptr,
                               0u, vars_per_bin, (uint32_t)n_vars, (uint32_t)n_layers, d_nbdds, (REAL*)nullptr, d_delta_lay, RunStep{}, al);
        }
        delta_var_valid = false;
        prof_end(BDDMMA_K_FINISH_DELTA);
    }
    int isotropic_dist_weights(void* out, int on_device) override
    {
        HIPCHK(hipSetDevice(device));
        REAL* dst = on_device ? (REAL*)out : d_tmp0;
        hipLaunchKernelGGL((k_isotropic_alpha<REAL>), dim3(cdiv(n_layers, 256)), dim3(256), 0, stream, d_var, d_nbdds, dst, (uint32_t)n_layers);
        HIPCHK(hipGetLastError());
        if (!on_device) return copy_out(out, dst, n_layers * sizeof(REAL), 0);
        HIPCHK(hipStreamSynchronize(stream));
        return BDDMMA_OK;
    }
    int load_layer_values(REAL* dst, const void* src, int on_dev, const char* what)
    {
        if (!on_dev) {
            const REAL* h = (const REAL*)src;
            for (uint64_t l = 0; l < n_layers; ++l)
                if (!(h[l] >= REAL(0) && h[l] < std::numeric_limits<REAL>::infinity())) {
                    err = std::string("learned_iterations: ") + what + "[" + std::to_string(l) + "] is negative or not finite";
                    return BDDMMA_ERR_INVALID_ARGUMENT;
                }
        }
        HIPCHK(hipMemcpyAsync(dst, src, n_layers * sizeof(REAL), on_dev ? hipMemcpyDeviceToDevice : hipMemcpyHostToDevice, stream));
        if (on_dev) {
            HIPCHK(hipMemsetAsync(d_counts, 0, sizeof(uint32_t), stream));
            hipLaunchKernelGGL((k_count_bad_weights<REAL>), dim3(cdiv(n_layers, 256)), dim3(256), 0, stream, (const REAL*)dst, d_counts, (uint32_t)n_layers);
            uint32_t bad = 0;
            HIPCHK(hipMemcpyAsync(&bad, d_counts, sizeof(uint32_t), hipMemcpyDeviceToHost, stream));
            HIPCHK(hipStreamSynchronize(stream));
            if (bad) {
                err = "learned_iterations: " + std::to_string(bad) + " of the " + what + " are negative or not finite";
                return BDDMMA_ERR_INVALID_ARGUMENT;
            }
        }
        return BDDMMA_OK;
    }
    int learned_iterations(const void* w, int w_dev, uint64_t num_itr, double omega, double slope, void* sol_avg, void* lb1_avg, void* lb2_avg,
                           uint64_t cfi, double beta_d, int out_dev, uint64_t* itr_done, const void* omega_vec, int ov_dev) override
    {
        HIPCHK(hipSetDevice(device));
        int rc;
        if (itr_done) *itr_done = 0;
        if (!w) { err = "learned_iterations: dist_weights is null"; return BDDMMA_ERR_INVALID_ARGUMENT; }
        if (cfi > 0 && (!sol_avg || !lb1_avg || !lb2_avg)) {
            err = "learned_iterations: compute_history_for_itr > 0 needs sol_avg, lb_first_diff_avg and lb_second_diff_avg";
            return BDDMMA_ERR_INVALID_ARGUMENT;
        }
        if (*lbfgs_attached > 0) {
            err = "learned_iterations: an L-BFGS wrapper is attached to this solver (destroy it first: its history would not describe the costs any more)";
            return BDDMMA_ERR_STATE;
        }
        if (run_stop) { err = "learned_iterations: run_solver is queueing iterations"; return BDDMMA_ERR_STATE; }
        if (!d_alpha_ent && (rc = dalloc(&d_alpha_ent, n_layers))) return rc;
        const bool ov = omega_vec != nullptr;
        if (ov) {
            if (!ov_ready) {
                if ((rc = ov_prepare())) return rc;
                ov_ready = true;
            }
// ... 314 lines not shown
        HIPCHK(hipSetDevice(device));
        int rc = elem_precision == BDDMMA_F64 ? update_both<double>(lo, n_lo, hi, n_hi, on_device) : update_both<float>(lo, n_lo, hi, n_hi, on_device);
        if (rc) return rc;
        costs_changed();
        HIPCHK(hipGetLastError());
        return BDDMMA_OK;
    }
    int set_cost(double c, uint64_t var) override
    {
        if (var >= n_vars) { err = "variable out of range"; return BDDMMA_ERR_INVALID_ARGUMENT; }
        HIPCHK(hipSetDevice(device));
        const uint32_t k0 = h_var_ptr[var], k1 = h_var_ptr[var + 1];
        if (k1 > k0) {
            const REAL cc = REAL(c / (double)(k1 - k0));
            hipLaunchKernelGGL((k_set_cost<REAL>), dim3(cdiv(k1 - k0, 64)), dim3(64), 0, stream, d_hi, d_var_layers, k0, k1, cc);
        }
        costs_changed();
        HIPCHK(hipGetLastError());
        return BDDMMA_OK;
    }
    int copy_out(void* dst, const void* src, size_t bytes, int on_device) const
    {
        std::string& err = const_cast<std::string&>(this->err);
        if (!dst) return BDDMMA_OK;
        HIPCHK(hipMemcpyAsync(dst, src, bytes, on_device ? hipMemcpyDeviceToDevice : hipMemcpyDeviceToHost, stream));
        HIPCHK(hipStreamSynchronize(stream));
        return BDDMMA_OK;
    }
    int get_solver_costs(void* lo, void* hi, void* mm, int on_device) override
    {
        int rc;
        std::string& err = const_cast<std::string&>(this->err);
        HIPCHK(hipSetDevice(device));
        const dim3 g(cdiv(n_layers, 256)), b(256);
        if (lo) {
            hipLaunchKernelGGL((k_strided_copy<REAL>), g, b, 0, stream, d_tmp0, 1u, (const REAL*)d_lo, 2u, (uint32_t)n_layers);
            if ((rc = copy_out(lo, d_tmp0, n_layers * sizeof(REAL), on_device))) return rc;
        }
        if (hi) {
            hipLaunchKernelGGL((k_strided_copy<REAL>), g, b, 0, stream, d_tmp0, 1u, (const REAL*)d_hi, 2u, (uint32_t)n_layers);
            if ((rc = copy_out(hi, d_tmp0, n_layers * sizeof(REAL), on_device))) return rc;
        }
        if (!mm) return BDDMMA_OK;
        hipLaunchKernelGGL((k_entries_to_layers<REAL>), dim3(cdiv(n_layers, 256)), dim3(256), 0, stream, d_mm_binned, d_lpos, d_tmp0, (uint32_t)n_layers);
        return copy_out(mm, d_tmp0, n_layers * sizeof(REAL), on_device);
    }
    int set_solver_costs(const void* lo, const void* hi, const void* mm, int on_device) override
    {
        const hipMemcpyKind k = on_device ? hipMemcpyDeviceToDevice : hipMemcpyHostToDevice;
        HIPCHK(hipSetDevice(device));
        const dim3 g(cdiv(n_layers, 256)), b(256);
        if (lo) {
            HIPCHK(hipMemcpyAsync(d_tmp0, lo, n_layers * sizeof(REAL), k, stream));
            hipLaunchKernelGGL((k_strided_copy<REAL>), g, b, 0, stream, d_lo, 2u, (const REAL*)d_tmp0, 1u, (uint32_t)n_layers);
        }
        if (hi) {
            HIPCHK(hipMemcpyAsync(d_tmp0, hi, n_layers * sizeof(REAL), k, stream));
            hipLaunchKernelGGL((k_strided_copy<REAL>), g, b, 0, stream, d_hi, 2u, (const REAL*)d_tmp0, 1u, (uint32_t)n_layers);
        }
        if (mm) {
            x_layer_valid = false;
            HIPCHK(hipMemcpyAsync(d_tmp0, mm, n_layers * sizeof(REAL), k, stream));
            hipLaunchKernelGGL((k_layers_to_entries<REAL>), dim3(cdiv(n_layers, 256)), dim3(256), 0, stream, d_tmp0, d_lpos, d_mm_binned, (uint32_t)n_layers);
        }
        HIPCHK(hipStreamSynchronize(stream));
        costs_changed();
        return BDDMMA_OK;
    }
    int primal_objective_vec(void* out, int on_device) override
    {
        HIPCHK(hipSetDevice(device));
        REAL* dst = on_device ? (REAL*)out : d_delta_c;
        hipLaunchKernelGGL((k_primal_objective<REAL>), dim3(cdiv(n_vars, 256)), dim3(256), 0, stream, d_lo, d_hi, d_var_ptr, d_var_layers, dst, (uint32_t)n_vars);
        if (!on_device) return copy_out(out, dst, n_vars * sizeof(REAL), 0);
        HIPCHK(hipStreamSynchronize(stream));
        return BDDMMA_OK;
    }
    int min_marginals(int sorted, int32_t* var, void* mm0, void* mm1, int on_device) override
    {
        HIPCHK(hipSetDevice(device));
        int rc;
        if ((rc = forward_run())) return rc;
        if ((rc = launch_bwd(BWD_MARGINALS, nullptr, REAL(0), BDDMMA_K_OTHER))) return rc;
        bwd_valid = true;
        return marginals_out(sorted, var, mm0, mm1, on_device);
    }
    int marginals_out(int sorted, int32_t* var, void* mm0, void* mm1, int on_device)
    {
        const hipMemcpyKind k = on_device ? hipMemcpyDeviceToDevice : hipMemcpyDeviceToHost;
        if (!sorted) {
            if (var) HIPCHK(hipMemcpyAsync(var, d_var, n_layers * sizeof(int32_t), k, stream));
            if (mm0) HIPCHK(hipMemcpyAsync(mm0, d_tmp0, n_layers * sizeof(REAL), k, stream));
            if (mm1) HIPCHK(hipMemcpyAsync(mm1, d_tmp1, n_layers * sizeof(REAL), k, stream));
            HIPCHK(hipStreamSynchronize(stream));
            return BDDMMA_OK;
        }
        REAL *s0 = nullptr, *s1 = nullptr;
        int32_t* sv = nullptr;
        HIPCHK(hipMalloc((void**)&s0, std::max<uint64_t>(n_layers, 1) * sizeof(REAL)));
        HIPCHK(hipMalloc((void**)&s1, std::max<uint64_t>(n_layers, 1) * sizeof(REAL)));
        HIPCHK(hipMalloc((void**)&sv, std::max<uint64_t>(n_layers, 1) * sizeof(int32_t)));
        const dim3 g(cdiv(n_layers, 256)), b(256);
        hipLaunchKernelGGL((k_gather<REAL>), g, b, 0, stream, d_tmp0, d_var_layers, s0, (uint32_t)n_layers);
        hipLaunchKernelGGL((k_gather<REAL>), g, b, 0, stream, d_tmp1, d_var_layers, s1, (uint32_t)n_layers);
        hipLaunchKernelGGL(k_gather_var, g, b, 0, stream, d_var, d_var_layers, sv, (uint32_t)n_layers);
        hipError_t e = hipSuccess;
        if (var && e == hipSuccess) e = hipMemcpyAsync(var, sv, n_layers * sizeof(int32_t), k, stream);
        if (mm0 && e == hipSuccess) e = hipMemcpyAsync(mm0, s0, n_layers * sizeof(REAL), k, stream);
        if (mm1 && e == hipSuccess) e = hipMemcpyAsync(mm1, s1, n_layers * sizeof(REAL), k, stream);
        if (e == hipSuccess) e = hipStreamSynchronize(stream);
        (void)hipFree(s0); (void)hipFree(s1); (void)hipFree(sv);
        HIPCHK(e);
        return BDDMMA_OK;
    }
    template <typename... TAIL, typename... ARGS>
    int launch_pull(const PullSweep<REAL, TAIL...>& s, ARGS... tail)
    {
        const DevPtrs<REAL> d = ptrs(nullptr);
        auto family = [&](auto fn, const PackBufs& b, uint32_t lb_base, uint32_t threads, uint32_t ww, const uint32_t* ptr, const uint32_t* par, unsigned char* scratch) {
            if (!b.n_packs) return;
            prof_begin(BDDMMA_K_OTHER);
            hipLaunchKernelGGL(fn, dim3(b.n_packs), dim3(threads), scratch ? 0 : s.bytes(sizeof(REAL), ww), stream, d, pdev(b, lb_base), ptr, par, ww, scratch, tail...);
            prof_end(BDDMMA_K_OTHER);
        };
        family(s.narrow, nb_, 0, 64, pack_width, d_sm_nptr, d_sm_npar, nullptr);
        family(s.wide, wb_, nb_.n_packs, WIDE_THREADS, wide_pack_width, d_sm_wptr, d_sm_wpar, nullptr);
        family(s.huge, hb_, nb_.n_packs + wb_.n_packs, WIDE_THREADS, huge_pack_width, d_sm_wptr, d_sm_wpar, s.scratch);
        HIPCHK(hipGetLastError());
        return BDDMMA_OK;
    }
    template <typename... A, typename... B>
    int pull_wide_lds(const char* what, const PullSweep<REAL, A...>& a, const PullSweep<REAL, B...>& b)
    {
        const uint32_t wl = (uint32_t)a.bytes(sizeof(REAL), wide_pack_width);
        if (wb_.n_packs && wl > lds_cu) { err = std::string(what) + ": a wide pack does not fit the LDS"; return BDDMMA_ERR_UNSUPPORTED; }
        if (wb_.n_packs && wl > 48 * 1024) {
            HIPCHK(hipFuncSetAttribute(reinterpret_cast<const void*>(a.wide), hipFuncAttributeMaxDynamicSharedMemorySize, (int)wl));
            HIPCHK(hipFuncSetAttribute(reinterpret_cast<const void*>(b.wide), hipFuncAttributeMaxDynamicSharedMemorySize, (int)wl));
        }
        return BDDMMA_OK;
    }
    PullSweep<REAL> sm_fwd_sweep() const, sm_bwd_sweep() const;
    int sm_prepare();
    int sm_launch_fwd();
    int sm_launch_bwd();
    int sm_sum_marginals(int sorted, int log_probs, int32_t* var, void* sm0, void* sm1, int on_device);
    int sm_smooth_solution(void* out, int on_device);
    bool sm_ready = false;
    uint32_t *d_sm_nptr = nullptr, *d_sm_npar = nullptr, *d_sm_wptr = nullptr, *d_sm_wpar = nullptr;
    unsigned char* d_sm_scratch = nullptr;
    int sum_marginals(int sorted, int log_probs, int32_t* var, void* sm0, void* sm1, int on_device) override
    {
        return sm_sum_marginals(sorted, log_probs, var, sm0, sm1, on_device);
    }
    int smooth_solution(void* out, int on_device) override { return sm_smooth_solution(out, on_device); }
    PullSweep<REAL, const REAL*, REAL*, REAL*, uint32_t*> gr_down_sweep() const;
    PullSweep<REAL, const REAL*, REAL*, REAL*, const uint32_t*> gr_up_sweep() const;
    int gr_prepare();
    int gr_inputs(bool second);
    int gr_launch_down();
    int gr_launch_up();
    int gr_load(REAL* dst, const void* src, uint64_t n, int on_dev, const char* what);
    struct LoadSpec { REAL* dst; const void* src; const char* what; bool weights; };
    int gr_load_device(const LoadSpec* specs, int count, uint64_t n, const char* me);
    int gr_min_marginal_diff(const void* grad_mm, void* grad_lo, void* grad_hi, int on_device);
    int gr_lower_bound_per_bdd(const void* grad_lb, void* grad_lo, void* grad_hi, int smooth, int on_device);
    int gr_distribute_delta(const void* grad_lo, const void* grad_hi, void* grad_deferred_mm, int on_device);
    int gr_cost_perturbation(const void* grad_lo, const void* grad_hi, void* grad_lo_pert, void* grad_hi_pert, int on_device);
    bool gr_ready = false;
    REAL *d_gr_in0 = nullptr, *d_gr_in1 = nullptr;
    uint32_t* d_gr_arg = nullptr;
    unsigned char* d_gr_scratch = nullptr;
    REAL* d_mm_consumed = nullptr;
    bool mm_consumed_valid = false;
    int grad_min_marginal_diff(const void* g, void* lo, void* hi, int on_device) override { return gr_min_marginal_diff(g, lo, hi, on_device); }
    int grad_lower_bound_per_bdd(const void* g, void* lo, void* hi, int smooth, int on_device) override { return gr_lower_bound_per_bdd(g, lo, hi, smooth, on_device); }
    int grad_distribute_delta(const void* lo, const void* hi, void* out, int on_device) override { return gr_distribute_delta(lo, hi, out, on_device); }
    int grad_cost_perturbation(const void* lo, const void* hi, void* lo_p, void* hi_p, int on_device) override { return gr_cost_perturbation(lo, hi, lo_p, hi_p, on_device); }
    int gi_prepare(uint64_t n_caches);
    int gi_grad_learned_iterations(const void* w, int w_dev, double omega, const void* omega_vec, int ov_dev, void* grad_lo, void* grad_hi, void* grad_mm,
                                   void* grad_w_out, void* grad_omega_out, uint64_t after, uint64_t n, uint64_t num_caches, int on_device);
    int gi_time_kernel(int kind, uint64_t reps, double* ms);
    struct { int kind = 0; uint64_t reps = 0; float ms = 0.f; } gi_timing;
    bool gi_ready = false;
    REAL* d_gi = nullptr;
    std::vector<REAL*> gi_caches;
    unsigned char* d_gi_scratch = nullptr;
    int grad_learned_iterations(const void* w, int w_dev, double omega, const void* omega_vec, int ov_dev, void* grad_lo, void* grad_hi, void* grad_mm,
                                void* grad_w_out, void* grad_omega_out, uint64_t after, uint64_t n, uint64_t num_caches, int on_device) override
    {
        return gi_grad_learned_iterations(w, w_dev, omega, omega_vec, ov_dev, grad_lo, grad_hi, grad_mm, grad_w_out, grad_omega_out, after, n, num_caches, on_device);
    }
    int min_marginal_diff(void* out, int on_device) override
    {
        HIPCHK(hipSetDevice(device));
        int rc;
        if ((rc = forward_run())) return rc;
        if ((rc = launch_bwd(BWD_MARGINALS, nullptr, REAL(0), BDDMMA_K_OTHER))) return rc;
        bwd_valid = true;
        REAL* dst = on_device ? (REAL*)out : d_tmp0;
        hipLaunchKernelGGL((k_diff<REAL, REAL>), dim3(cdiv(n_layers, 256)), dim3(256), 0, stream, dst, (const REAL*)d_tmp1, (const REAL*)d_tmp0, (uint32_t)n_layers);
        if (!on_device) return copy_out(out, dst, n_layers * sizeof(REAL), 0);
        HIPCHK(hipStreamSynchronize(stream));
        return BDDMMA_OK;
    }
    int bdds_solution(int sorted, char* sol, int on_device) override
    {
        HIPCHK(hipSetDevice(device));
        int rc;
        if ((rc = backward_run())) return rc;
        HIPCHK(hipMemsetAsync(d_sol, 0, n_layers, stream));
        if ((rc = launch_fwd(FWD_SOLUTION, nullptr, REAL(0), BDDMMA_K_OTHER))) return rc;
        const hipMemcpyKind k = on_device ? hipMemcpyDeviceToDevice : hipMemcpyDeviceToHost;
        if (!sorted) {
            HIPCHK(hipMemcpyAsync(sol, d_sol, n_layers, k, stream));
            HIPCHK(hipStreamSynchronize(stream));
            return BDDMMA_OK;
        }
        char* s = nullptr;
        HIPCHK(hipMalloc((void**)&s, std::max<uint64_t>(n_layers, 1)));
        hipLaunchKernelGGL((k_gather<char>), dim3(cdiv(n_layers, 256)), dim3(256), 0, stream, d_sol, d_var_layers, s, (uint32_t)n_layers);
        hipError_t e = hipMemcpyAsync(sol, s, n_layers, k, stream);
        if (e == hipSuccess) e = hipStreamSynchronize(stream);
        (void)hipFree(s);
        HIPCHK(e);
        return BDDMMA_OK;
    }
    int bdds_solution_async(char* dev_out, int prezeroed) override
    {
        HIPCHK(hipSetDevice(device));
        int rc;
        if ((rc = backward_run())) return rc;
        if (!prezeroed) HIPCHK(hipMemsetAsync(dev_out, 0, n_layers, stream));
        char* const own = d_sol;
        d_sol = dev_out;
        rc = launch_fwd(FWD_SOLUTION, nullptr, REAL(0), BDDMMA_K_OTHER);
        d_sol = own;
        if (rc) return rc;
        return BDDMMA_OK;
    }
    int lbfgs_views(LbfgsViews* out) override
    {
        HIPCHK(hipSetDevice(device));
        int rc;
        if (!d_x_layer && (rc = dalloc(&d_x_layer, n_layers))) return rc;
        if (!x_layer_valid) {
            hipLaunchKernelGGL((k_net_costs<REAL>), dim3(cdiv(n_layers, 256)), dim3(256), 0, stream, d_lo, d_hi, d_mm_binned, d_lpos, d_x_layer, (uint32_t)n_layers);
            HIPCHK(hipGetLastError());
            x_layer_valid = true;
        }
        *out = LbfgsViews{d_x_layer};
        return BDDMMA_OK;
    }
    int net_solver_costs(void* out, int on_device) override
    {
        HIPCHK(hipSetDevice(device));
        REAL* dst = on_device ? (REAL*)out : d_tmp0;
        hipLaunchKernelGGL((k_net_costs<REAL>), dim3(cdiv(n_layers, 256)), dim3(256), 0, stream, d_lo, d_hi, d_mm_binned, d_lpos, dst, (uint32_t)n_layers);
        if (!on_device) return copy_out(out, dst, n_layers * sizeof(REAL), 0);
        HIPCHK(hipGetLastError());
        return BDDMMA_OK;
    }
    int make_dual_feasible(void* g, int on_device) override
    {
        HIPCHK(hipSetDevice(device));
        REAL* p = (REAL*)g;
        if (!on_device) { p = d_tmp0; HIPCHK(hipMemcpyAsync(p, g, n_layers * sizeof(REAL), hipMemcpyHostToDevice, stream)); }
        hipLaunchKernelGGL((k_make_dual_feasible<REAL>), dim3(cdiv(n_vars, 256)), dim3(256), 0, stream, p, d_var_ptr, d_var_layers, (uint32_t)n_vars);
        if (!on_device) return copy_out(g, p, n_layers * sizeof(REAL), 0);
        HIPCHK(hipGetLastError());
        return BDDMMA_OK;
    }
    int gradient_step(const void* g, double step, int on_device) override
    {
        HIPCHK(hipSetDevice(device));
        const REAL* p = (const REAL*)g;
        if (!on_device) { HIPCHK(hipMemcpyAsync(d_tmp0, g, n_layers * sizeof(REAL), hipMemcpyHostToDevice, stream)); p = d_tmp0; }
        hipLaunchKernelGGL((k_gradient_step<REAL>), dim3(cdiv(n_layers, 256)), dim3(256), 0, stream, d_hi, p, REAL(step), (uint32_t)n_layers);
        costs_changed();
        HIPCHK(hipGetLastError());
        return BDDMMA_OK;
    }
// ... 26 lines not shown
        HIPCHK(hipSetDevice(device));
        int rc;
        proj_staged = use_staged_projection();
        proj_pending = false;
        proj_of = g;
        if (!proj_staged) {
            if (!d_proj_q && (rc = dalloc(&d_proj_q, n_vars))) return rc;
            hipLaunchKernelGGL((k_projection_means<REAL>), dim3(cdiv(n_vars, 256)), dim3(256), 0, stream, (const REAL*)g, d_var_ptr, d_var_layers, d_proj_q, (uint32_t)n_vars);
            HIPCHK(hipGetLastError());
            return BDDMMA_OK;
        }
        if (!d_proj_dir && (rc = dalloc(&d_proj_dir, n_layers))) return rc;
        if (!d_proj_ent && (rc = dalloc(&d_proj_ent, n_layers))) return rc;
        launch_stage_transpose(0, (const REAL*)g, d_proj_ent, (REAL*)nullptr, REAL(0));
        if (n_layers > n_narrow_layers)
            hipLaunchKernelGGL((k_layers_to_entries<REAL>), dim3(cdiv(n_layers - n_narrow_layers, 256)), dim3(256), 0, stream, (const REAL*)g + n_narrow_layers,
                               d_lpos + n_narrow_layers, d_proj_ent, (uint32_t)(n_layers - n_narrow_layers));
        launch_project_entries();
        HIPCHK(hipGetLastError());
        return BDDMMA_OK;
    }
    bool projection_fuses_lincomb() const override { return use_staged_projection() && n_layers == n_narrow_layers && !(opts_variant & 0x8000u); }
    int projection_means_lincomb(const LinComb& lc, const void* tag) override
    {
        HIPCHK(hipSetDevice(device));
        int rc;
        if (!projection_fuses_lincomb() || lc.ns < 1 || lc.ns > LINCOMB_MAX) { err = "projection_means_lincomb: not available for this instance"; return BDDMMA_ERR_INVALID_ARGUMENT; }
        proj_staged = true;
        proj_pending = false;
        proj_of = tag;
        if (!d_proj_dir && (rc = dalloc(&d_proj_dir, n_layers))) return rc;
        if (!d_proj_ent && (rc = dalloc(&d_proj_ent, n_layers))) return rc;
        const Kern<LincombFn>& k = kern.lincomb[lc.ns == 5];
        hipLaunchKernelGGL(k.fn, dim3(cdiv(nb_.n_packs, wpb)), dim3(64 * wpb), k.lds, stream, lc, d_proj_ent, pdev(nb_, 0), (const uint32_t*)d_cs_entry,
                           (const uint16_t*)d_cs_slot, n_narrow_layers, (uint32_t)n_layers);
        launch_project_entries();
        HIPCHK(hipGetLastError());
        return BDDMMA_OK;
    }
    int gradient_step_projected(const void* g, double step) override
    {
        HIPCHK(hipSetDevice(device));
        if (g != proj_of) { err = "gradient_step_projected: not the vector projection_means was called on"; return BDDMMA_ERR_INVALID_ARGUMENT; }
        if (proj_staged) {
            if (proj_pending) {
                launch_stage_transpose(1, (const REAL*)d_proj_ent, d_proj_dir, d_lohi, REAL(step));
                if (n_layers > n_narrow_layers) {
                    const uint32_t nw = (uint32_t)(n_layers - n_narrow_layers);
                    hipLaunchKernelGGL((k_entries_to_layers<REAL>), dim3(cdiv(nw, 256)), dim3(256), 0, stream, (const REAL*)d_proj_ent, d_lpos + n_narrow_layers,
                                       d_proj_dir + n_narrow_layers, nw);
                    hipLaunchKernelGGL((k_gradient_step<REAL>), dim3(cdiv(nw, 256)), dim3(256), 0, stream, d_hi + 2 * (size_t)n_narrow_layers,
                                       (const REAL*)d_proj_dir + n_narrow_layers, REAL(step), nw);
                }
                proj_pending = false;
            } else {
                hipLaunchKernelGGL((k_gradient_step<REAL>), dim3(cdiv(n_layers, 256)), dim3(256), 0, stream, d_hi, (const REAL*)d_proj_dir, REAL(step), (uint32_t)n_layers);
            }
            costs_changed();
            HIPCHK(hipGetLastError());
            return BDDMMA_OK;
        }
        if (!d_proj_q) { err = "gradient_step_projected without projection_means"; return BDDMMA_ERR_INVALID_ARGUMENT; }
        hipLaunchKernelGGL((k_gradient_step_projected<REAL>), dim3(cdiv(n_layers, 256)), dim3(256), 0, stream, d_hi, (const REAL*)g, d_proj_q, (const uint32_t*)d_var, REAL(step), (uint32_t)n_layers);
        costs_changed();
        HIPCHK(hipGetLastError());
        return BDDMMA_OK;
    }
    void* stream_handle() override { return (void*)stream; }
    int rounding_scratch(void** c0_dev, void** c1_dev) override
    {
        *c0_dev = d_delta_c;
        *c1_dev = d_delta_c + n_vars;
        return BDDMMA_OK;
    }
    int rounding_round(double delta, uint32_t round, uint32_t seed, uint32_t counts[4], char* sol_host, void* c0_host, void* c1_host,
                       bool apply_update, int* applied) override
    {
        HIPCHK(hipSetDevice(device));
        int rc;
        *applied = 0;
        if ((rc = distribute_delta())) return rc;
        if ((rc = forward_run())) return rc;
        if ((rc = launch_bwd(BWD_MARGINALS, nullptr, REAL(0), BDDMMA_K_OTHER))) return rc;
        bwd_valid = true;
        HIPCHK(hipMemsetAsync(d_counts, 0, 4 * sizeof(uint32_t), stream));
        REAL* c0 = d_delta_c;
        REAL* c1 = d_delta_c + n_vars;
        hipLaunchKernelGGL((k_round_perturb<REAL>), dim3(cdiv(n_vars, 256)), dim3(256), 0, stream, d_tmp0, d_tmp1, d_var_ptr, d_var_layers,
                           c0, c1, d_sol, d_counts, (uint32_t)n_vars, delta, round, seed);
        HIPCHK(hipMemcpyAsync(counts, d_counts, 4 * sizeof(uint32_t), hipMemcpyDeviceToHost, stream));
        if (c0_host) HIPCHK(hipMemcpyAsync(c0_host, c0, n_vars * sizeof(REAL), hipMemcpyDeviceToHost, stream));
        if (c1_host) HIPCHK(hipMemcpyAsync(c1_host, c1, n_vars * sizeof(REAL), hipMemcpyDeviceToHost, stream));
        HIPCHK(hipStreamSynchronize(stream));
        if ((uint64_t)counts[0] + counts[1] == n_vars) {
            HIPCHK(hipMemcpyAsync(sol_host, d_sol, n_vars, hipMemcpyDeviceToHost, stream));
            HIPCHK(hipStreamSynchronize(stream));
            return BDDMMA_OK;
        }
        *applied = 1;
        if (!apply_update) return BDDMMA_OK;
        return update_costs(c0, n_vars, c1, n_vars, precision, 1);
    }
    int time_stream(bool copy, uint64_t reps, double* ms)
    {
        const uint64_t n4 = BDDMMA_TRIAD_BYTES / 16;
        stream_v4 *a = nullptr, *b = nullptr, *c = nullptr;
        HIPCHK(hipMalloc(&a, BDDMMA_TRIAD_BYTES));
        HIPCHK(hipMalloc(&b, BDDMMA_TRIAD_BYTES));
        HIPCHK(hipMalloc(&c, BDDMMA_TRIAD_BYTES));
        HIPCHK(hipMemsetAsync(b, 0, BDDMMA_TRIAD_BYTES, stream));
        HIPCHK(hipMemsetAsync(c, 0, BDDMMA_TRIAD_BYTES, stream));
        const unsigned grid = (unsigned)((n4 + 255) / 256);
        auto once = [&]() {
            if (copy) k_stream<true><<<grid, 256, 0, stream>>>(a, b, c, 3.0f, n4);
            else k_stream<false><<<grid, 256, 0, stream>>>(a, b, c, 3.0f, n4);
        };
        once();
        HIPCHK(hipEventRecord(ev_t0, stream));
        for (uint64_t i = 0; i < reps; ++i) once();
        HIPCHK(hipEventRecord(ev_t1, stream));
        HIPCHK(hipEventSynchronize(ev_t1));
        float f = 0.f;
        HIPCHK(hipEventElapsedTime(&f, ev_t0, ev_t1));
        *ms = f;
        HIPCHK(hipFree(a));
        HIPCHK(hipFree(b));
        HIPCHK(hipFree(c));
        return BDDMMA_OK;
    }

    int time_kernel(int kind, uint64_t reps, double* ms) override
    {
        HIPCHK(hipSetDevice(device));
        if (kind >= 13 && kind <= 17) return gi_time_kernel(kind, reps, ms);
        int rc = BDDMMA_OK;
        auto once = [&]() -> int {
            switch (kind) {
                case 0: return launch_fwd(FWD_PLAIN, nullptr, REAL(0), BDDMMA_K_OTHER);
                case 1: return launch_bwd(BWD_PLAIN, nullptr, REAL(0), BDDMMA_K_OTHER);
                case 2: return launch_fwd(FWD_SOLVE, d_delta_lay, REAL(0.5), BDDMMA_K_OTHER);
                case 3: return launch_bwd(BWD_SOLVE, d_delta_lay, REAL(0.5), BDDMMA_K_OTHER);
                case 4: return exchange();
                case 5: launch_bcast(d_delta_c, d_delta_lay_c); return BDDMMA_OK;
                case 8: return sm_launch_fwd();
                case 9: return sm_launch_bwd();
                case 10: return gr_launch_down();
                case 11: return gr_launch_up();
                case 12: { const int r = gr_launch_down(); return r ? r : gr_launch_up(); }
                default: err = "unknown kernel kind"; return BDDMMA_ERR_INVALID_ARGUMENT;
            }
        };
        if (kind == 6 || kind == 7) return time_stream(kind == 7, reps, ms);
        if ((kind == 8 || kind == 9) && (rc = sm_prepare())) return rc;
        if (kind == 9 && (rc = sm_launch_fwd())) return rc;
        if (kind >= 10 && kind <= 12) {
            if ((rc = gr_prepare()) || (rc = forward_run()) || (rc = backward_run())) return rc;
            HIPCHK(hipMemsetAsync(d_gr_in0, 0, n_layers * sizeof(REAL), stream));
            if (kind == 11 && (rc = gr_launch_down())) return rc;
        }
        if ((rc = once())) return rc;
        HIPCHK(hipEventRecord(ev_t0, stream));
        for (uint64_t i = 0; i < reps; ++i)
            if ((rc = once())) return rc;
        HIPCHK(hipEventRecord(ev_t1, stream));
        HIPCHK(hipEventSynchronize(ev_t1));
        float f = 0.f;
        HIPCHK(hipEventElapsedTime(&f, ev_t0, ev_t1));
// ... 33 lines not shown
```

bdd_amd/csrc/solver_sm.hpp:

```cpp
#pragma once
#include "solver_impl.hpp"
#include "kernels/summarg.hpp"

namespace bddmma {

struct SmPackSet {
    std::vector<uint32_t> pack_hop_ptr, hop_node_off;
};
template <typename WORD, typename DECODE, typename WORDOF>
static bool sm_build_parents(const std::vector<SmPackSet>& sets, const std::vector<WORD>& words, DECODE decode, WORDOF word_of, std::vector<uint32_t>& ptr,
                             std::vector<uint32_t>& par)
{
    const size_t nw = words.size();
    ptr.assign(nw + 1, 0);
    std::vector<uint8_t> seen(nw, 0);
    for (int pass = 0; pass < 2; ++pass) {
        std::vector<uint32_t> fill;
        if (pass == 1) {
            for (size_t i = 0; i < nw; ++i) ptr[i + 1] += ptr[i];
            par.assign(ptr[nw], 0);
            fill.assign(ptr.begin(), ptr.end() - 1);
            std::fill(seen.begin(), seen.end(), 0);
        }
        for (const SmPackSet& ps : sets)
// ... 28 lines not shown
{
    if (sm_ready) return BDDMMA_OK;
    HIPCHK(hipSetDevice(device));
    auto fetch = [&](int id, auto& vec) -> hipError_t {
        using T = typename std::remove_reference_t<decltype(vec)>::value_type;
        const DevField& f = dev_fields[id];
        vec.resize(f.count);
        return f.count ? hipMemcpyAsync(vec.data(), f.ptr, f.count * sizeof(T), hipMemcpyDeviceToHost, stream) : hipSuccess;
    };
    int rc;
    if (nb_.n_packs) {
        std::vector<uint32_t> words, word_off;
        std::vector<SmPackSet> sets(1);
        HIPCHK(fetch(LAY_NARROW_WORDS, words)); HIPCHK(fetch(LAY_NARROW_WORD_OFF, word_off));
        HIPCHK(fetch(LAY_NARROW_PACK_HOP_PTR, sets[0].pack_hop_ptr)); HIPCHK(fetch(LAY_NARROW_HOP_NODE_OFF, sets[0].hop_node_off));
        HIPCHK(hipStreamSynchronize(stream));
        std::vector<uint32_t> ptr, par;
        const uint32_t W = pack_width;
        const bool ok = sm_build_parents(sets, words,
                         [W](uint32_t w, uint32_t (&ch)[2]) {
                             if (w & NW_PAD) return false;
                             ch[0] = w & NW_CHILD_MASK;
                             ch[1] = (w >> NW_CHILD_BITS) & NW_CHILD_MASK;
                             if (ch[0] >= W) ch[0] = 0xFFFFFFFFu;
                             if (ch[1] >= W) ch[1] = 0xFFFFFFFFu;
                             return true;
                         },
                         [&](const SmPackSet&, size_t p) { return (size_t)word_off[p]; }, ptr, par);
        if (!ok) { err = "sum-marginals: a narrow pack's node words lie outside the word array"; return BDDMMA_ERR_STATE; }
        if ((rc = upload(&d_sm_nptr, ptr))) return rc;
        if ((rc = upload(&d_sm_npar, par))) return rc;
        HIPCHK(hipStreamSynchronize(stream));
    }
    if (wb_.n_packs || hb_.n_packs) {
        std::vector<uint64_t> words;
        HIPCHK(fetch(LAY_WIDE_WORDS, words));
        std::vector<SmPackSet> sets(2);
        HIPCHK(fetch(LAY_WIDE_PACK_HOP_PTR, sets[0].pack_hop_ptr)); HIPCHK(fetch(LAY_WIDE_HOP_NODE_OFF, sets[0].hop_node_off));
        HIPCHK(fetch(LAY_HUGE_PACK_HOP_PTR, sets[1].pack_hop_ptr)); HIPCHK(fetch(LAY_HUGE_HOP_NODE_OFF, sets[1].hop_node_off));
        HIPCHK(hipStreamSynchronize(stream));
        std::vector<uint32_t> ptr, par;
        const uint32_t wsb = wide_slot_base;
        const bool ok = sm_build_parents(sets, words,
                         [](uint64_t w, uint32_t (&ch)[2]) {
                             const uint64_t lo = w & WW_CHILD_MASK, hi = (w >> WW_CHILD_BITS) & WW_CHILD_MASK;
                             ch[0] = lo < WW_TOP ? (uint32_t)lo : 0xFFFFFFFFu;
                             ch[1] = hi < WW_TOP ? (uint32_t)hi : 0xFFFFFFFFu;
                             return true;
                         },
                         [&](const SmPackSet& ps, size_t p) { return (size_t)(ps.hop_node_off[ps.pack_hop_ptr[p]] - wsb); }, ptr, par);
        if (!ok) { err = "sum-marginals: a wide pack's node words lie outside the word array"; return BDDMMA_ERR_STATE; }
        if ((rc = upload(&d_sm_wptr, ptr))) return rc;
        if ((rc = upload(&d_sm_wpar, par))) return rc;
        HIPCHK(hipStreamSynchronize(stream));
    }
    if (hb_.n_packs && (rc = dalloc(&d_sm_scratch, (uint64_t)hb_.n_packs * sm_lds_bytes(sizeof(REAL), huge_pack_width)))) return rc;
    if ((rc = pull_wide_lds("sum-marginals", sm_fwd_sweep(), sm_bwd_sweep()))) return rc;
    sm_ready = true;
    return BDDMMA_OK;
}

template <typename REAL>
PullSweep<REAL> SolverT<REAL>::sm_fwd_sweep() const
{
    return {&k_sm_fwd<REAL, true, false>, &k_sm_fwd<REAL, false, false>, &k_sm_fwd<REAL, false, true>, &sm_lds_bytes, d_sm_scratch};
}
template <typename REAL>
PullSweep<REAL> SolverT<REAL>::sm_bwd_sweep() const
{
    return {&k_sm_bwd<REAL, true, false>, &k_sm_bwd<REAL, false, false>, &k_sm_bwd<REAL, false, true>, &sm_lds_bytes, d_sm_scratch};
}

template <typename REAL>
int SolverT<REAL>::sm_launch_fwd()
{
    if (int rc = launch_pull(sm_fwd_sweep())) return rc;
    fwd_valid = false;
    return BDDMMA_OK;
}

template <typename REAL>
int SolverT<REAL>::sm_launch_bwd()
{
    bwd_valid = false;
    lb_cached = false;
    ++lb_gen;
    return launch_pull(sm_bwd_sweep());
}

template <typename REAL>
int SolverT<REAL>::sm_sum_marginals(int sorted, int log_probs, int32_t* var, void* sm0, void* sm1, int on_device)
{
    HIPCHK(hipSetDevice(device));
    int rc;
    if ((rc = sm_prepare())) return rc;
    if ((rc = sm_launch_fwd())) return rc;
    if ((rc = sm_launch_bwd())) return rc;
    if (!log_probs) hipLaunchKernelGGL((k_exp_pair<REAL>), dim3(cdiv(n_layers, 256)), dim3(256), 0, stream, d_tmp0, d_tmp1, (uint32_t)n_layers);
    return marginals_out(sorted, var, sm0, sm1, on_device);
}

template <typename REAL>
int SolverT<REAL>::sm_smooth_solution(void* out, int on_device)
{
    HIPCHK(hipSetDevice(device));
    int rc;
    if ((rc = sm_prepare())) return rc;
    if ((rc = sm_launch_fwd())) return rc;
    if ((rc = sm_launch_bwd())) return rc;
    REAL* dst = on_device ? (REAL*)out : d_tmp0;
    hipLaunchKernelGGL((k_smooth_solution<REAL>), dim3(cdiv(n_layers, 256)), dim3(256), 0, stream, (const REAL*)d_tmp0, (const REAL*)d_tmp1, dst, (uint32_t)n_layers);
    if (!on_device) return copy_out(out, dst, n_layers * sizeof(REAL), 0);
    HIPCHK(hipStreamSynchronize(stream));
    return BDDMMA_OK;
}

}
```

bdd_amd/solver.py:

```python
from __future__ import annotations

import ctypes as C

import numpy as np

from . import capi
from .bdd_collection import BddCollection


def _ptr(a):
    return a.ctypes.data_as(C.c_void_p) if a is not None else None


def _is_dev(x):
    return hasattr(x, "data_ptr") and bool(getattr(x, "is_cuda", False))


def _dev_ptr(x, n, dtype):
    assert x.is_contiguous() and x.numel() >= n, "device buffer too small or not contiguous"
    assert x.element_size() == np.dtype(dtype).itemsize, "device buffer has the wrong element type"
    return C.c_void_p(x.data_ptr())


class bdd_hip_parallel_mma:

    def __init__(self, bdd_col: BddCollection, costs_hi=None, precision: str = "double", device: int = 0,
                 pack_width: int = 0, wide_pack_width: int = 0, deterministic: bool = False,
                 vars_per_bin: int = 0, stage_cap: int = 0, waves_per_block: int = 0, keep_bdd_order: bool = False,
                 resident_sweeps: int = 0, exchange_by_variable: int = 0, variant_flags: int = 0, pack_fill: int = 0, pack_stagger: int = 0, _handle=None):
        self._L = capi.lib()
        self.value_type = {"double": np.float64, "float": np.float32, "single": np.float32}[precision]
        self._prec = capi.F64 if self.value_type == np.float64 else capi.F32
        if _handle is not None:
            self._h = _handle
            return
        instr = np.ascontiguousarray(bdd_col.instr, dtype=np.uint64)
        delims = np.ascontiguousarray(bdd_col.delims, dtype=np.uint64)
        opts = capi.Options(pack_width, wide_pack_width, 1 if deterministic else 0, vars_per_bin, stage_cap, waves_per_block)
        opts.keep_bdd_order = int(keep_bdd_order)
        opts.resident_sweeps = int(resident_sweeps)
        opts.exchange_by_variable = int(exchange_by_variable)
        opts.pack_fill = int(pack_fill)
        opts.pack_stagger = int(pack_stagger)
        opts.variant_flags = int(variant_flags)
        h = C.c_void_p()
        costs = None if costs_hi is None else np.ascontiguousarray(costs_hi, dtype=np.float64)
        rc = self._L.bddmma_create(C.byref(h), self._prec, device, _ptr(instr), _ptr(delims), bdd_col.nr_bdds(),
                                   _ptr(costs), 0 if costs is None else costs.size, C.byref(opts))
        capi.check(rc, None)
        self._h = h

    def close(self):
        if getattr(self, "_h", None):
            self._L.bddmma_destroy(self._h)
            self._h = None

    def __del__(self):
        try:
            self.close()
        except Exception:
            pass

    def _ck(self, rc):
        capi.check(rc, self._h)

    def nr_variables(self): return int(self._L.bddmma_nr_variables(self._h))
    def nr_layers(self): return int(self._L.bddmma_nr_layers(self._h))
    def nr_bdd_nodes(self): return int(self._L.bddmma_nr_bdd_nodes(self._h))
    def nr_hops(self): return int(self._L.bddmma_nr_hops(self._h))
    def nr_packs(self): return int(self._L.bddmma_nr_packs(self._h))

    SWEEP_KINDS = ("none", "mixed", "streaming1", "streaming2", "streaming3", "resident1", "resident2")

    def solve_sweep_kind(self) -> str:
        return self.SWEEP_KINDS[int(self._L.bddmma_solve_sweep_kind(self._h))]
    def fused_small(self) -> bool:
        return bool(self._L.bddmma_fused_small(self._h))
    def fused_small_learned(self) -> bool:
        return bool(self._L.bddmma_fused_small_learned(self._h))

    def nontemporal_loads(self) -> bool:
        return bool(self._L.bddmma_nontemporal_loads(self._h))
    def device(self) -> int:
        return int(self._L.bddmma_device(self._h))
    def device_bytes(self): return int(self._L.bddmma_device_bytes(self._h))
    def device_allocated_bytes(self): return int(self._L.bddmma_device_allocated_bytes(self._h))

    def nr_bdds(self, var=None):
        if var is None:
            return int(self._L.bddmma_nr_bdds(self._h))
        return int(self.get_num_bdds_per_var()[var])

    def get_num_bdds_per_var(self):
        out = np.zeros(self.nr_variables(), np.int32)
        self._ck(self._L.bddmma_num_bdds_per_var(self._h, _ptr(out)))
        return out

    def get_primal_variable_index(self):
        out = np.zeros(self.nr_layers(), np.int32)
        self._ck(self._L.bddmma_layer_variables(self._h, _ptr(out)))
        return out

    def get_bdd_index(self):
        out = np.zeros(self.nr_layers(), np.int32)
        self._ck(self._L.bddmma_layer_bdds(self._h, _ptr(out)))
        return out

    def nodes_per_hop(self):
        out = np.zeros(self.nr_hops(), np.uint64)
        self._ck(self._L.bddmma_nodes_per_hop(self._h, _ptr(out)))
        return out

    def layers_per_hop(self):
        out = np.zeros(self.nr_hops(), np.uint64)
        self._ck(self._L.bddmma_layers_per_hop(self._h, _ptr(out)))
        return out

    def bdd_major_order(self):
        return np.argsort(self.get_bdd_index(), kind="stable")

    def update_costs(self, cost_delta_0, cost_delta_1):
        if _is_dev(cost_delta_0) or _is_dev(cost_delta_1):
            n0 = cost_delta_0.numel() if cost_delta_0 is not None else 0
            n1 = cost_delta_1.numel() if cost_delta_1 is not None else 0
            self._ck(self._L.bddmma_update_costs(self._h, _dev_ptr(cost_delta_0, n0, self.value_type) if n0 else None, n0,
                                                 _dev_ptr(cost_delta_1, n1, self.value_type) if n1 else None, n1, self._prec, 1))
            return
        lo = np.ascontiguousarray(cost_delta_0, dtype=np.float64)
        hi = np.ascontiguousarray(cost_delta_1, dtype=np.float64)
        self._ck(self._L.bddmma_update_costs(self._h, _ptr(lo), lo.size, _ptr(hi), hi.size, capi.F64, 0))

    def set_cost(self, c, var):
        self._ck(self._L.bddmma_set_cost(self._h, float(c), int(var)))

    def get_solver_costs(self, out=None):
        n = self.nr_layers()
        if out is not None:
            self._ck(self._L.bddmma_get_solver_costs(self._h, *(_dev_ptr(x, n, self.value_type) for x in out), 1))
            return out
        lo, hi, mm = (np.zeros(n, self.value_type) for _ in range(3))
        self._ck(self._L.bddmma_get_solver_costs(self._h, _ptr(lo), _ptr(hi), _ptr(mm), 0))
        return lo, hi, mm

    def set_solver_costs(self, lo, hi, mm):
        if _is_dev(lo):
            n = self.nr_layers()
            self._ck(self._L.bddmma_set_solver_costs(self._h, *(_dev_ptr(x, n, self.value_type) for x in (lo, hi, mm)), 1))
            return
        lo, hi, mm = (np.ascontiguousarray(x, dtype=self.value_type) for x in (lo, hi, mm))
        self._ck(self._L.bddmma_set_solver_costs(self._h, _ptr(lo), _ptr(hi), _ptr(mm), 0))

    def get_primal_objective_vector(self, out):
        self._ck(self._L.bddmma_primal_objective_vec(self._h, _dev_ptr(out, self.nr_variables(), self.value_type), 1))
        return out

    def get_primal_objective_vector_host(self):
        out = np.zeros(self.nr_variables(), self.value_type)
        self._ck(self._L.bddmma_primal_objective_vec(self._h, _ptr(out), 0))
        return out

    def forward_run(self): self._ck(self._L.bddmma_forward_run(self._h))
    def backward_run(self): self._ck(self._L.bddmma_backward_run(self._h))

    def lower_bound(self) -> float:
        lb = C.c_double()
# ... 492 lines not shown
```

include/bdd_mma.h:

```cpp
#ifndef BDD_MMA_H
#define BDD_MMA_H

#include <stddef.h>
#include <stdint.h>

#ifdef __cplusplus
extern "C" {
#endif

#define BDDMMA_OK 0
#define BDDMMA_ERR_INVALID_ARGUMENT (-1)
#define BDDMMA_ERR_INVALID_BDD (-2)
#define BDDMMA_ERR_DEVICE (-3)
#define BDDMMA_ERR_STATE (-4)
#define BDDMMA_ERR_UNSUPPORTED (-5)
#define BDDMMA_ERR_IO (-6)

#define BDDMMA_F32 0
#define BDDMMA_F64 1

typedef struct bddmma_instruction {
    uint64_t lo;
    uint64_t hi;
    uint64_t index;
} bddmma_instruction;

#define BDDMMA_TOPSINK UINT64_MAX
#define BDDMMA_BOTSINK (UINT64_MAX - 1)

typedef struct bddmma_solver bddmma_solver;

typedef struct bddmma_options {
    uint32_t pack_width;
    uint32_t wide_pack_width;
    uint32_t deterministic;
    uint32_t vars_per_bin;
    uint32_t stage_cap;
    uint32_t waves_per_block;
    uint32_t keep_bdd_order;
    uint32_t resident_sweeps;
    uint32_t exchange_by_variable;
    uint32_t variant_flags;
    uint32_t pack_fill;
    uint32_t pack_stagger;
} bddmma_options;


int bddmma_create(bddmma_solver** out, int precision, int device,
                  const bddmma_instruction* instr, const uint64_t* bdd_delims, uint64_t n_bdds,
                  const double* costs_hi, uint64_t n_costs, const bddmma_options* opts);
void bddmma_destroy(bddmma_solver* s);

int bddmma_device_count(void);
int bddmma_device_chip(int device, uint32_t* n_cus, uint32_t* lds_bytes_per_cu, uint64_t* max_resident_threads);
int bddmma_set_layout_threads(int n);
int bddmma_set_thread_layout_threads(int n);
const char* bddmma_last_error(const bddmma_solver* s);

uint64_t bddmma_nr_variables(const bddmma_solver* s);
uint64_t bddmma_nr_bdds(const bddmma_solver* s);
uint64_t bddmma_nr_layers(const bddmma_solver* s);
uint64_t bddmma_nr_bdd_nodes(const bddmma_solver* s);
uint64_t bddmma_nr_hops(const bddmma_solver* s);
uint64_t bddmma_nr_packs(const bddmma_solver* s);
enum {
    BDDMMA_SWEEPS_NONE = 0,
    BDDMMA_SWEEPS_MIXED = 1,
    BDDMMA_SWEEPS_STREAMING1 = 2,
    BDDMMA_SWEEPS_STREAMING2 = 3,
    BDDMMA_SWEEPS_STREAMING3 = 4,
    BDDMMA_SWEEPS_RESIDENT1 = 5,
    BDDMMA_SWEEPS_RESIDENT2 = 6
};
int bddmma_solve_sweep_kind(const bddmma_solver* s);
int bddmma_fused_small(const bddmma_solver* s);
int bddmma_fused_small_learned(const bddmma_solver* s);
int bddmma_nontemporal_loads(const bddmma_solver* s);
int bddmma_precision(const bddmma_solver* s);
int bddmma_device(const bddmma_solver* s);
int bddmma_num_bdds_per_var(const bddmma_solver* s, int32_t* out);
int bddmma_layer_variables(const bddmma_solver* s, int32_t* out);
int bddmma_layer_bdds(const bddmma_solver* s, int32_t* out);
int bddmma_nodes_per_hop(const bddmma_solver* s, uint64_t* out);
int bddmma_layers_per_hop(const bddmma_solver* s, uint64_t* out);

int bddmma_update_costs(bddmma_solver* s, const void* lo, uint64_t n_lo, const void* hi, uint64_t n_hi,
                        int elem_precision, int on_device);
int bddmma_set_cost(bddmma_solver* s, double c, uint64_t var);
int bddmma_get_solver_costs(const bddmma_solver* s, void* lo, void* hi, void* deferred_mm_diff, int on_device);
int bddmma_set_solver_costs(bddmma_solver* s, const void* lo, const void* hi, const void* deferred_mm_diff, int on_device);
int bddmma_primal_objective_vec(bddmma_solver* s, void* out, int on_device);

int bddmma_forward_run(bddmma_solver* s);
int bddmma_backward_run(bddmma_solver* s);
int bddmma_lower_bound(bddmma_solver* s, double* lb);
int bddmma_lower_bound_per_bdd(bddmma_solver* s, void* out, int on_device);

int bddmma_iteration(bddmma_solver* s, double omega);
int bddmma_iterations(bddmma_solver* s, double omega, uint64_t n);
int bddmma_forward_mm(bddmma_solver* s, double omega, void* delta_lo_hi, int on_device);
int bddmma_backward_mm(bddmma_solver* s, double omega, void* delta_lo_hi, int on_device);
int bddmma_normalize_delta(const bddmma_solver* s, void* delta_lo_hi, int on_device);
int bddmma_distribute_delta(bddmma_solver* s);
int bddmma_get_delta(const bddmma_solver* s, void* out, int on_device);
int bddmma_set_delta(bddmma_solver* s, const void* in, int on_device);

int bddmma_learned_iterations(bddmma_solver* s, const void* dist_weights, int weights_on_device, uint64_t num_itr, double omega,
                              double improvement_slope, void* sol_avg, void* lb_first_diff_avg, void* lb_second_diff_avg,
                              uint64_t compute_history_for_itr, double history_avg_beta, int outputs_on_device, uint64_t* itr_done);
int bddmma_learned_iterations_omega_vec(bddmma_solver* s, const void* dist_weights, int weights_on_device, uint64_t num_itr, const void* omega_vec,
                                        int omega_vec_on_device, double improvement_slope, void* sol_avg, void* lb_first_diff_avg,
                                        void* lb_second_diff_avg, uint64_t compute_history_for_itr, double history_avg_beta, int outputs_on_device,
                                        uint64_t* itr_done);
int bddmma_isotropic_dist_weights(bddmma_solver* s, void* out, int on_device);

int bddmma_min_marginals(bddmma_solver* s, int sorted, int32_t* var, void* mm0, void* mm1, int on_device);
int bddmma_min_marginal_diff(bddmma_solver* s, void* out, int on_device);
int bddmma_sum_marginals(bddmma_solver* s, int sorted, int log_probs, int32_t* var, void* sm0, void* sm1, int on_device);
int bddmma_smooth_solution(bddmma_solver* s, void* out, int on_device);
int bddmma_bdds_solution(bddmma_solver* s, int sorted, char* sol, int on_device);

int bddmma_grad_min_marginal_diff(bddmma_solver* s, const void* grad_mm, void* grad_lo_out, void* grad_hi_out, int on_device);
int bddmma_grad_lower_bound_per_bdd(bddmma_solver* s, const void* grad_lb_per_bdd, void* grad_lo_out, void* grad_hi_out, int smooth, int on_device);
int bddmma_grad_distribute_delta(bddmma_solver* s, const void* grad_lo, const void* grad_hi, void* grad_deferred_mm_out, int on_device);
int bddmma_grad_cost_perturbation(bddmma_solver* s, const void* grad_lo, const void* grad_hi, void* grad_lo_pert_out, void* grad_hi_pert_out, int on_device);

int bddmma_grad_learned_iterations(bddmma_solver* s, const void* dist_weights, int weights_on_device, double omega, const void* omega_vec,
                                   int omega_vec_on_device, void* grad_lo, void* grad_hi, void* grad_mm, void* grad_dist_weights_out, void* grad_omega_out,
                                   uint64_t track_grad_after_itr, uint64_t track_grad_for_num_itr, uint64_t num_caches, int on_device);

int bddmma_net_solver_costs(const bddmma_solver* s, void* out, int on_device);
int bddmma_make_dual_feasible(const bddmma_solver* s, void* g, int on_device);
int bddmma_gradient_step(bddmma_solver* s, const void* g, double step_size, int on_device);

typedef struct bddmma_lbfgs bddmma_lbfgs;
typedef struct bddmma_lbfgs_params {
    int32_t history_size;
    double init_step_size;
    double req_rel_lb_increase;
    double step_size_decrease_factor;
    double step_size_increase_factor;
} bddmma_lbfgs_params;
int bddmma_lbfgs_create(bddmma_lbfgs** out, bddmma_solver* s, const bddmma_lbfgs_params* p);
void bddmma_lbfgs_destroy(bddmma_lbfgs* l);
int bddmma_lbfgs_iteration(bddmma_lbfgs* l);
int bddmma_lbfgs_update_costs(bddmma_lbfgs* l, const void* lo, uint64_t n_lo, const void* hi, uint64_t n_hi,
                              int elem_precision, int on_device);
int bddmma_lbfgs_flush(bddmma_lbfgs* l);
typedef struct bddmma_lbfgs_state {
    double step_size;
    double last_applied_step;
    uint64_t mma_iterations;
    uint64_t lbfgs_iterations;
    int32_t history_entries;
    int32_t num_unsuccessful_updates;
    int32_t last_kind;
    int32_t last_trials;
} bddmma_lbfgs_state;
int bddmma_lbfgs_get_state(const bddmma_lbfgs* l, bddmma_lbfgs_state* out);

// ... 82 lines not shown
```

Baseline: 8777.

## Add narrow4 sweep kernels that rebuild potentials on chip instead of HBM round-trip

Adds new forward/backward narrow sweep kernels that can rebuild the opposite-direction potentials (T or F) in LDS at the start of each pack rather than reading them from global memory, and optionally skip storing them. Solver state tracking gains a separate lb_valid flag so a sweep that does not persist potentials still leaves the lower bound usable, and the MMA iteration path selects these on-chip sweeps when usable. This trades extra recomputation and LDS work per pack for less HBM traffic in a bandwidth-bound solver, with added state-validity complexity.

```diff
diff --git a/bdd_amd/capi.py b/bdd_amd/capi.py
--- a/bdd_amd/capi.py
+++ b/bdd_amd/capi.py
@@ -59,6 +59,7 @@
     "bddmma_fused_small": (_I, [_V]),
     "bddmma_fused_small_learned": (_I, [_V]),
     "bddmma_nontemporal_loads": (_I, [_V]),
+    "bddmma_potentials_on_chip": (_I, [_V]),
     "bddmma_precision": (_I, [_V]),
     "bddmma_device": (_I, [_V]),
     "bddmma_num_bdds_per_var": (_I, [_V, _V]),
diff --git a/bdd_amd/csrc/capi.cpp b/bdd_amd/csrc/capi.cpp
--- a/bdd_amd/csrc/capi.cpp
+++ b/bdd_amd/csrc/capi.cpp
@@ -155,6 +155,7 @@
 int bddmma_fused_small(const bddmma_solver* s) { return s && s->impl ? (s->impl->fused_small ? 1 : 0) : -1; }
 int bddmma_fused_small_learned(const bddmma_solver* s) { return s && s->impl ? (s->impl->fused_small_learned ? 1 : 0) : -1; }
 int bddmma_nontemporal_loads(const bddmma_solver* s) { return s && s->impl ? (s->impl->nt_loads ? 1 : 0) : -1; }
+int bddmma_potentials_on_chip(const bddmma_solver* s) { return s && s->impl ? (s->impl->pot_on_chip ? 1 : 0) : -1; }
 int bddmma_precision(const bddmma_solver* s) { return s && s->impl ? s->impl->precision : -1; }
 int bddmma_device(const bddmma_solver* s) { return s && s->impl ? s->impl->device : -1; }
 uint64_t bddmma_device_bytes(const bddmma_solver* s) { return s && s->impl ? s->impl->dev_bytes : 0; }
diff --git a/bdd_amd/csrc/kernels.hpp b/bdd_amd/csrc/kernels.hpp
--- a/bdd_amd/csrc/kernels.hpp
+++ b/bdd_amd/csrc/kernels.hpp
@@ -12,6 +12,7 @@
 #include "kernels/resident.hpp"
 #include "kernels/narrow2.hpp"
 #include "kernels/narrow3.hpp"
+#include "kernels/narrow4.hpp"
 #include "kernels/wide.hpp"
 #include "kernels/exchange.hpp"
 #include "kernels/small.hpp"
diff --git a/bdd_amd/csrc/kernels/narrow4.hpp b/bdd_amd/csrc/kernels/narrow4.hpp
--- /dev/null
+++ b/bdd_amd/csrc/kernels/narrow4.hpp
@@ -0,0 +1,348 @@
+#pragma once
+
+namespace bddmma {
+
+template <typename REAL, int WPB, int HC, bool REBUILD_T, bool STORE_F>
+__device__ __forceinline__ void fwd_narrow4_body(const DevPtrs<REAL>& d, const PackDev& pk, const uint32_t* __restrict__ lrec,
+                                                 const uint32_t* __restrict__ lrec_off, uint32_t lrec_words, REAL omega, uint32_t block_id)
+{
+    static_assert(HC + 1 <= (int)HOP_WIN, "one window of hop offsets has to hold the pack");
+    constexpr int W = N3_W;
+    constexpr uint32_t S = sizeof(REAL);
+    constexpr uint32_t BUF = (W + 128) * S;
+    using P2 = typename Pair<REAL>::type;
+    extern __shared__ __attribute__((aligned(16))) unsigned char dyn_lds[];
+    P2* sD = reinterpret_cast<P2*>(dyn_lds);
+    __shared__ __attribute__((aligned(16))) unsigned char sF_[WPB][2][BUF];
+    __shared__ __attribute__((aligned(16))) unsigned char sT_[WPB][2][BUF];
+    __shared__ uint32_t sOffN_[WPB][HOP_WIN], sOffL_[WPB][HOP_WIN], sOffR_[WPB][HOP_WIN];
+    const uint32_t tid = threadIdx.x;
+    const int wave = __builtin_amdgcn_readfirstlane((int)(tid >> 6));
+    const int lane = tid & 63;
+    unsigned char* sFw = &sF_[wave][0][0];
+    unsigned char* sTw = &sT_[wave][0][0];
+    const uint32_t n_quads = (pk.n_packs + WPB - 1) / WPB;
+    const uint32_t quad = block_to_pack(block_id, n_quads, pk.xcd_chunk);
+    BDDMMA_EXIT_IF(quad >= n_quads, d)
+    const uint32_t p = quad * WPB + wave;
+    const bool has_pack = p < pk.n_packs;
+    const uint32_t* const hp = pk.hdr_pack + 8 * (size_t)(has_pack ? p : 0);
+    const uint32_t q0 = !has_pack ? 0 : hp[4];
+    const uint32_t hops = !has_pack ? 0 : (hp[5] & 0xFFFFu);
+    const uint32_t q1 = q0 + hops;
+    const uint32_t rbase = has_pack ? lrec_off[p] : 0;
+    const uint32_t c0_h = pk.hdr_quad[4 * (size_t)quad], cnt = pk.hdr_quad[4 * (size_t)quad + 1];
+    BDDMMA_STAMP(p, 0);
+    const REAL INF = inf_v<REAL>();
+    const uint32_t slot_first = !has_pack ? 0 : hp[0], l0 = !has_pack ? 0 : hp[2];
+    NarrowRs<REAL> rs(d);
+    rs.rebase_layers(d, l0);
+    uint32_t ent[STAGE_ITERS], esl[STAGE_ITERS];
+    stage_load_tables<REAL, WPB, BDDMMA_LD_TAB_AUX>(ent, esl, rs, c0_h, cnt, tid);
+    REAL* const Tp = d.T + slot_first;
+    REAL* const Fp = d.F + slot_first;
+    const REAL* const lohi_p = d.lohi + 2 * (size_t)l0;
+    const rsrc_t rr = make_rsrc(lrec, lrec_words);
+    HopWindow hw{sOffN_[wave], sOffL_[wave], sOffR_[wave], q0, q1, slot_first, l0};
+    uint32_t o[HC + 4];
+    uint32_t lb[HC + 1];
+    P2 L[HC];
+    P2 T[HC + 2];
+#pragma unroll
+    for (int i = 0; i < HC + 4; ++i) o[i] = 0;
+#pragma unroll
+    for (int i = 0; i < HC + 1; ++i) lb[i] = 0;
+#pragma unroll
+    for (int i = 0; i < HC + 2; ++i) T[i] = P2{REAL(0), REAL(0)};
+    auto ldrec = [&](uint32_t h) { return __builtin_amdgcn_raw_buffer_load_b128(rr, (uint32_t)lane * 16u, (rbase + h * 64u) * 16u, 0); };
+    const uint32_t sink = (W + 2 * (uint32_t)lane) * S;
+    u4v rA = u4v{0u, 0u, 0u, 0u}, rB = rA;
+    const uint32_t db = (uint32_t)wave * pk.stage_cap * (uint32_t)sizeof(P2);
+    if (has_pack) {
+        hw.fill(pk, q0, lane);
+#pragma unroll
+        for (int i = 0; i < HC + 4; ++i) o[i] = hw.node_off(q0 + i);
+#pragma unroll
+        for (int i = 0; i < HC + 1; ++i) lb[i] = hw.layer_off(q0 + i);
+#pragma unroll
+        for (int h = 0; h < HC; ++h)
+            hop_load(L[h], rs.lohi, (uint32_t)h < hops ? (uint32_t)lane * (uint32_t)sizeof(P2) : OOB, lb[h] * (uint32_t)sizeof(P2));
+        if constexpr (!REBUILD_T) {
+#pragma unroll
+            for (int h = 1; h < HC; ++h) pot_pair_load<REAL, false>(T[h], hop_rsrc(Tp, o[h], o[h + 1] - o[h]), 2u * (uint32_t)lane * S, o[h] * S);
+        }
+#pragma unroll
+        for (int r = 0; r < 2; ++r) {
+            const uint32_t j = lane + 64 * r;
+            lds_st<REAL>(sFw, j * S, (j < o[1] - o[0]) ? REAL(0) : INF);
+        }
+#pragma unroll
+        for (int b = 0; b < 2; ++b) {
+            lds_st<REAL>(sTw, b * BUF + sink, REAL(0));
+            lds_st<REAL>(sTw, b * BUF + sink + S, INF);
+        }
+        wave_sync();
+        if constexpr (REBUILD_T) {
+            rA = ldrec(hops - 1);
+            rB = ldrec(hops >= 2 ? hops - 2 : 0);
+#pragma unroll
+            for (int h = HC - 1; h >= 1; --h) {
+                if ((uint32_t)h < hops) {
+                    const u4v ra = rA;
+                    rA = rB;
+                    rB = ldrec(h >= 2 ? h - 2 : 0);
+                    const uint32_t tc = ((h + 1) & 1) * BUF, tn = (h & 1) * BUF;
+                    const P2 c = L[h];
+                    const uint32_t flags = ra[2] >> 16;
+                    const REAL tla = lds_ld<REAL>(sTw, tc + (ra[0] & 0xFFFFu)), tha = lds_ld<REAL>(sTw, tc + (ra[0] >> 16));
+                    const REAL tlb = lds_ld<REAL>(sTw, tc + (ra[1] & 0xFFFFu)), thb = lds_ld<REAL>(sTw, tc + (ra[1] >> 16));
+                    const REAL ta = rmin(c.y + tha, c.x + tla);
+                    const REAL tb = rmin(c.y + thb, c.x + tlb);
+                    if (flags & LREC_REAL) lds_st<REAL>(sTw, tn + (ra[2] & 0xFFFFu), ta);
+                    if (flags & LREC_TWO) lds_st<REAL>(sTw, tn + (ra[2] & 0xFFFFu) + S, tb);
+                    wave_sync();
+                    T[h] = lds_ld<P2>(sTw, tn + 2u * (uint32_t)lane * S);
+                }
+            }
+        } else {
+            if (2u * (uint32_t)lane < o[2] - o[1]) lds_st<P2>(sTw, BUF + 2u * (uint32_t)lane * S, T[1]);
+        }
+        rA = ldrec(0);
+        rB = ldrec(1);
+    }
+    stage_load_pairs<REAL, WPB>(sD, ent, esl, rs, cnt, tid);
+    if (WPB > 1) __syncthreads(); else wave_sync();
+    BDDMMA_STAMP(p, 1);
+#pragma unroll
+    for (int h = 0; h < HC; ++h) {
+        if ((uint32_t)h < hops) {
+            const u4v ra = rA;
+            rA = rB;
+            rB = ldrec(h + 2);
+            const uint32_t fc = (h & 1) * BUF, fn = ((h + 1) & 1) * BUF;
+            const uint32_t stg = db + (lb[h] + (uint32_t)lane) * (uint32_t)sizeof(P2);
+            const P2 c = L[h];
+            const uint32_t flags = ra[2] >> 16;
+            REAL fa, fb;
+            lds_ld2(fa, fb, sFw, fc + (ra[2] & 0xFFFFu));
+            const REAL tla = lds_ld<REAL>(sTw, fn + (ra[0] & 0xFFFFu)), tha = lds_ld<REAL>(sTw, fn + (ra[0] >> 16));
+            const REAL tlb = lds_ld<REAL>(sTw, fn + (ra[1] & 0xFFFFu)), thb = lds_ld<REAL>(sTw, fn + (ra[1] >> 16));
+            const P2 dd = lds_ld<P2>(dyn_lds, stg);
+            if (!(REBUILD_T && h == 0))
+                if (2u * (uint32_t)lane < o[h + 3] - o[h + 2]) lds_st<P2>(sTw, fc + 2u * (uint32_t)lane * S, T[h + 2]);
+            lds_st<P2>(sFw, fn + 2u * (uint32_t)lane * S, P2{INF, INF});
+            wave_sync();
+            fa = (flags & LREC_REAL) ? fa : INF;
+            fb = (flags & LREC_TWO) ? fb : INF;
+            const REAL m0 = rmin((fa + c.x) + tla, (fb + c.x) + tlb);
+            const REAL m1 = rmin((fa + c.y) + tha, (fb + c.y) + thb);
+            const REAL mm = mm_diff1(m0, m1, omega);
+            P2 nc;
+            nc.x = (c.x + min0(mm)) + dd.x;
+            nc.y = (c.y + min0_neg(mm)) + dd.y;
+            const rsrc_t rl = hop_rsrc(reinterpret_cast<const P2*>(lohi_p), lb[h], lb[h + 1] - lb[h]);
+            hop_store(nc, rl, (uint32_t)lane * (uint32_t)sizeof(P2), lb[h] * (uint32_t)sizeof(P2));
+            if (flags & LREC_REAL) lds_st<REAL>(dyn_lds, stg, mm);
+            lds_min(reinterpret_cast<REAL*>(sFw + fn + (ra[0] & 0xFFFFu)), fa + nc.x);
+            lds_min(reinterpret_cast<REAL*>(sFw + fn + (ra[0] >> 16)), fa + nc.y);
+            lds_min(reinterpret_cast<REAL*>(sFw + fn + (ra[1] & 0xFFFFu)), fb + nc.x);
+            lds_min(reinterpret_cast<REAL*>(sFw + fn + (ra[1] >> 16)), fb + nc.y);
+            if constexpr (STORE_F) {
+                const rsrc_t rf = hop_rsrc(Fp, o[h], o[h + 1] - o[h]);
+                pot_store_layer<REAL>(fa, fb, (flags & LREC_TWO) != 0, rf, ra[3] & 0xFFFFu, o[h] * S, pk.nt_potentials);
+            }
+            wave_sync();
+        }
+    }
+    BDDMMA_STAMP(p, 3);
+    if (WPB > 1) __syncthreads(); else wave_sync();
+    BDDMMA_STAMP(p, 2);
+    stage_flush<REAL, WPB>(sD, ent, esl, rs, cnt, tid);
+    BDDMMA_STAMP(p, 4);
+}
+
+template <typename REAL, int WPB, int HC, bool REBUILD_T, bool STORE_F>
+__global__ void __launch_bounds__(64 * WPB) __attribute__((amdgpu_waves_per_eu(4))) k_fwd_narrow4(DevPtrs<REAL> d, PackDev pk, const uint32_t* __restrict__ lrec, const uint32_t* __restrict__ lrec_off,
+                                                          uint32_t lrec_words, REAL omega)
+{
+    fwd_narrow4_body<REAL, WPB, HC, REBUILD_T, STORE_F>(d, pk, lrec, lrec_off, lrec_words, omega, blockIdx.x);
+}
+
+template <typename REAL, int WPB, int HC, bool REBUILD_F, bool STORE_T>
+__device__ __forceinline__ void bwd_narrow4_body(const DevPtrs<REAL>& d, const PackDev& pk, const uint32_t* __restrict__ lrec,
+                                                 const uint32_t* __restrict__ lrec_off, uint32_t lrec_words, REAL omega, uint32_t block_id)
+{
+    static_assert(HC + 1 <= (int)HOP_WIN, "one window of hop offsets has to hold the pack");
+    constexpr int W = N3_W;
+    constexpr uint32_t S = sizeof(REAL);
+    constexpr uint32_t BUF = (W + 128) * S;
+    using P2 = typename Pair<REAL>::type;
+    extern __shared__ __attribute__((aligned(16))) unsigned char dyn_lds[];
+    P2* sD = reinterpret_cast<P2*>(dyn_lds);
+    __shared__ __attribute__((aligned(16))) unsigned char sT_[WPB][2][BUF];
+    __shared__ uint32_t sOffN_[WPB][HOP_WIN], sOffL_[WPB][HOP_WIN], sOffR_[WPB][HOP_WIN];
+    const uint32_t tid = threadIdx.x;
+    const int wave = __builtin_amdgcn_readfirstlane((int)(tid >> 6));
+    const int lane = tid & 63;
+    unsigned char* sTw = &sT_[wave][0][0];
+    const uint32_t n_quads = (pk.n_packs + WPB - 1) / WPB;
+    const uint32_t quad = block_to_pack(block_id, n_quads, pk.xcd_chunk);
+    BDDMMA_EXIT_IF(quad >= n_quads, d)
+    const uint32_t p = quad * WPB + wave;
+    const bool has_pack = p < pk.n_packs;
+    const uint32_t* const hp = pk.hdr_pack + 8 * (size_t)(has_pack ? p : 0);
+    const uint32_t q0 = !has_pack ? 0 : hp[4];
+    const uint32_t hops = !has_pack ? 0 : (hp[5] & 0xFFFFu);
+    const uint32_t q1 = q0 + hops;
+    const uint32_t rbase = has_pack ? lrec_off[p] : 0;
+    const uint32_t c0_h = pk.hdr_quad[4 * (size_t)quad], cnt = pk.hdr_quad[4 * (size_t)quad + 1];
+    BDDMMA_STAMP(p, 0);
+    const REAL INF = inf_v<REAL>();
+    const uint32_t slot_first = !has_pack ? 0 : hp[0], l0 = !has_pack ? 0 : hp[2];
+    NarrowRs<REAL> rs(d);
+    rs.rebase_layers(d, l0);
+    uint32_t ent[STAGE_ITERS], esl[STAGE_ITERS];
+    stage_load_tables<REAL, WPB, BDDMMA_LD_TAB_AUX>(ent, esl, rs, c0_h, cnt, tid);
+    REAL* const Tp = d.T + slot_first;
+    REAL* const Fp = d.F + slot_first;
+    const REAL* const lohi_p = d.lohi + 2 * (size_t)l0;
+    const rsrc_t rr = make_rsrc(lrec, lrec_words);
+    HopWindow hw{sOffN_[wave], sOffL_[wave], sOffR_[wave], q0, q1, slot_first, l0};
+    uint32_t o[HC + 1];
+    uint32_t lb[HC + 1];
+    P2 L[HC];
+    P2 F[HC];
+#pragma unroll
+    for (int i = 0; i < HC + 1; ++i) o[i] = lb[i] = 0;
+#pragma unroll
+    for (int i = 0; i < HC; ++i) F[i] = P2{REAL(0), REAL(0)};
+    auto ldrec = [&](uint32_t h) { return __builtin_amdgcn_raw_buffer_load_b128(rr, (uint32_t)lane * 16u, (rbase + h * 64u) * 16u, 0); };
+    const uint32_t sink = (W + 2 * (uint32_t)lane) * S;
+    u4v rA = u4v{0u, 0u, 0u, 0u}, rB = rA;
+    const uint32_t db = (uint32_t)wave * pk.stage_cap * (uint32_t)sizeof(P2);
+    if (has_pack) {
+        hw.fill(pk, q0, lane);
+#pragma unroll
+        for (int i = 0; i < HC + 1; ++i) {
+            o[i] = hw.node_off(q0 + i);
+            lb[i] = hw.layer_off(q0 + i);
+        }
+#pragma unroll
+        for (int h = 0; h < HC; ++h)
+            hop_load(L[h], rs.lohi, (uint32_t)h < hops ? (uint32_t)lane * (uint32_t)sizeof(P2) : OOB, lb[h] * (uint32_t)sizeof(P2));
+        if constexpr (REBUILD_F) {
+#pragma unroll
+            for (int r = 0; r < 2; ++r) {
+                const uint32_t j = lane + 64 * r;
+                lds_st<REAL>(sTw, j * S, (j < o[1] - o[0]) ? REAL(0) : INF);
+            }
+            rA = ldrec(0);
+            rB = ldrec(1);
+            wave_sync();
+#pragma unroll
+            for (int h = 0; h < HC; ++h) {
+                if ((uint32_t)h < hops) {
+                    const u4v ra = rA;
+                    rA = rB;
+                    rB = ldrec(h + 2);
+                    const uint32_t fc = (h & 1) * BUF, fn = ((h + 1) & 1) * BUF;
+                    const uint32_t flags = ra[2] >> 16;
+                    REAL fa, fb;
+                    lds_ld2(fa, fb, sTw, fc + (ra[2] & 0xFFFFu));
+                    F[h] = P2{fa, fb};
+                    if ((uint32_t)h + 1 < hops) {
+                        lds_st<P2>(sTw, fn + 2u * (uint32_t)lane * S, P2{INF, INF});
+                        wave_sync();
+                        const P2 c = L[h];
+                        fa = (flags & LREC_REAL) ? fa : INF;
+                        fb = (flags & LREC_TWO) ? fb : INF;
+                        lds_min(reinterpret_cast<REAL*>(sTw + fn + (ra[0] & 0xFFFFu)), fa + c.x);
+                        lds_min(reinterpret_cast<REAL*>(sTw + fn + (ra[0] >> 16)), fa + c.y);
+                        lds_min(reinterpret_cast<REAL*>(sTw + fn + (ra[1] & 0xFFFFu)), fb + c.x);
+                        lds_min(reinterpret_cast<REAL*>(sTw + fn + (ra[1] >> 16)), fb + c.y);
+                        wave_sync();
+                    }
+                }
+            }
+            wave_sync();
+        } else {
+#pragma unroll
+            for (int h = 0; h < HC; ++h) {
+                const uint32_t so = __builtin_amdgcn_raw_buffer_load_b32(rr, (uint32_t)lane * 16u + 12u, (rbase + ((uint32_t)h < hops ? h : 0u) * 64u) * 16u, 0);
+                pot_pair_load<REAL, false>(F[h], hop_rsrc(Fp, o[h], o[h + 1] - o[h]), so & 0xFFFFu, o[h] * S);
+            }
+        }
+#pragma unroll
+        for (int b = 0; b < 2; ++b) {
+            lds_st<REAL>(sTw, b * BUF + sink, REAL(0));
+            lds_st<REAL>(sTw, b * BUF + sink + S, INF);
+        }
+        rA = ldrec(hops - 1);
+        rB = ldrec(hops >= 2 ? hops - 2 : 0);
+        wave_sync();
+    }
+    stage_load_pairs<REAL, WPB>(sD, ent, esl, rs, cnt, tid);
+    if (WPB > 1) __syncthreads(); else wave_sync();
+    BDDMMA_STAMP(p, 1);
+#pragma unroll
+    for (int h = HC - 1; h >= 0; --h) {
+        if ((uint32_t)h < hops) {
+            const u4v ra = rA;
+            rA = rB;
+            rB = ldrec(h >= 2 ? h - 2 : 0);
+            const uint32_t tc = ((h + 1) & 1) * BUF, tn = (h & 1) * BUF;
+            const uint32_t stg = db + (lb[h] + (uint32_t)lane) * (uint32_t)sizeof(P2);
+            const P2 c = L[h];
+            const uint32_t flags = ra[2] >> 16;
+            const REAL tla = lds_ld<REAL>(sTw, tc + (ra[0] & 0xFFFFu)), tha = lds_ld<REAL>(sTw, tc + (ra[0] >> 16));
+            const REAL tlb = lds_ld<REAL>(sTw, tc + (ra[1] & 0xFFFFu)), thb = lds_ld<REAL>(sTw, tc + (ra[1] >> 16));
+            const P2 dd = lds_ld<P2>(dyn_lds, stg);
+            const REAL fa = (flags & LREC_REAL) ? F[h].x : INF;
+            const REAL fb = (flags & LREC_TWO) ? F[h].y : INF;
+            const REAL m0 = rmin((fa + c.x) + tla, (fb + c.x) + tlb);
+            const REAL m1 = rmin((fa + c.y) + tha, (fb + c.y) + thb);
+            const REAL mm = mm_diff1(m0, m1, omega);
+            P2 nc;
+            nc.x = (c.x + min0(mm)) + dd.x;
+            nc.y = (c.y + min0_neg(mm)) + dd.y;
+            const REAL ta = rmin(nc.y + tha, nc.x + tla);
+            const REAL tb = rmin(nc.y + thb, nc.x + tlb);
+            const rsrc_t rl = hop_rsrc(reinterpret_cast<const P2*>(lohi_p), lb[h], lb[h + 1] - lb[h]);
+            hop_store(nc, rl, (uint32_t)lane * (uint32_t)sizeof(P2), lb[h] * (uint32_t)sizeof(P2));
+            if (flags & LREC_REAL) {
+                lds_st<REAL>(dyn_lds, stg, mm);
+                lds_st<REAL>(sTw, tn + (ra[2] & 0xFFFFu), ta);
+            }
+            if (flags & LREC_TWO) lds_st<REAL>(sTw, tn + (ra[2] & 0xFFFFu) + S, tb);
+            if constexpr (STORE_T) {
+                const rsrc_t rt = hop_rsrc(Tp, o[h], o[h + 1] - o[h]);
+                pot_store_layer<REAL>(ta, tb, (flags & LREC_TWO) != 0, rt, ra[3] & 0xFFFFu, o[h] * S, pk.nt_potentials);
+            }
+            wave_sync();
+        }
+    }
+    BDDMMA_STAMP(p, 3);
+    if (WPB > 1) __syncthreads(); else wave_sync();
+    BDDMMA_STAMP(p, 2);
+    stage_flush<REAL, WPB>(sD, ent, esl, rs, cnt, tid);
+    BDDMMA_STAMP(p, 4);
+    if (!has_pack) return;
+    const uint32_t n0 = o[1] - o[0];
+    double s = 0.0;
+#pragma unroll
+    for (int r = 0; r < 2; ++r) {
+        const uint32_t j = lane + 64 * r;
+        if (j < n0) s += (double)lds_ld<REAL>(sTw, j * S);
+    }
+    for (int off2 = 32; off2 > 0; off2 >>= 1) s += __shfl_down(s, off2);
+    if (lane == 0) d.lb_partial[pk.lb_base + p] = s;
+}
+
+template <typename REAL, int WPB, int HC, bool REBUILD_F, bool STORE_T>
+__global__ void __launch_bounds__(64 * WPB) __attribute__((amdgpu_waves_per_eu(4))) k_bwd_narrow4(DevPtrs<REAL> d, PackDev pk, const uint32_t* __restrict__ lrec, const uint32_t* __restrict__ lrec_off,
+                                                          uint32_t lrec_words, REAL omega)
+{
+    bwd_narrow4_body<REAL, WPB, HC, REBUILD_F, STORE_T>(d, pk, lrec, lrec_off, lrec_words, omega, blockIdx.x);
+}
+
+}
diff --git a/bdd_amd/csrc/solver.hpp b/bdd_amd/csrc/solver.hpp
--- a/bdd_amd/csrc/solver.hpp
+++ b/bdd_amd/csrc/solver.hpp
@@ -23,6 +23,7 @@
     uint64_t dev_bytes = 0;
     uint64_t dev_alloc_bytes = 0;
     bool fwd_valid = false, bwd_valid = false;
+    bool lb_valid = false;
     uint64_t cost_epoch = 0;
     bool deterministic = false;
     std::vector<uint64_t> nodes_per_hop, layers_per_hop;
@@ -68,6 +69,7 @@
     bool fused_small = false;
     bool fused_small_learned = false;
     bool nt_loads = false;
+    bool pot_on_chip = false;
     virtual int run_plain(uint64_t max_iter, double tolerance, double slope, double time_limit, int verbose, bddmma_run_result* res) = 0;
     virtual int forward_mm(double omega, void* delta, int on_device) = 0;
     virtual int backward_mm(double omega, void* delta, int on_device) = 0;
diff --git a/bdd_amd/csrc/solver_bt.hpp b/bdd_amd/csrc/solver_bt.hpp
--- a/bdd_amd/csrc/solver_bt.hpp
+++ b/bdd_amd/csrc/solver_bt.hpp
@@ -626,7 +626,7 @@
             s->costs_changed();
             s->lb_cached = false;
             ++s->lb_gen;
-            s->bwd_valid = e == hipSuccess;
+            s->bwd_valid = s->lb_valid = e == hipSuccess;
         }
         const int rc2 = join_out();
         if (e != hipSuccess) { err = std::string("batch set_solver_costs: ") + hipGetErrorString(e); return BDDMMA_ERR_DEVICE; }
diff --git a/bdd_amd/csrc/solver_impl.hpp b/bdd_amd/csrc/solver_impl.hpp
--- a/bdd_amd/csrc/solver_impl.hpp
+++ b/bdd_amd/csrc/solver_impl.hpp
@@ -118,7 +118,7 @@
     bool x_layer_valid = false;
     void costs_changed()
     {
-        fwd_valid = bwd_valid = x_layer_valid = false;
+        fwd_valid = bwd_valid = lb_valid = x_layer_valid = false;
         ++cost_epoch;
     }
     CostQuot* d_cost_q = nullptr;
@@ -162,6 +162,8 @@
     SmallDev small_ln{};
     SmallLearn<REAL> small_ln_arg{};
     bool use_narrow3 = false;
+    int onchip_hc = 0;
+    uint32_t onchip_mode = 0;
     uint32_t *d_lrec = nullptr, *d_lrec_off = nullptr;
     uint32_t lrec_words = 0;
     uint32_t huge_pack_width = 0;
@@ -490,6 +492,20 @@
             n12_nt = false;
 #endif
         nt_loads = n3_nt || n12_nt;
+        if constexpr (sizeof(REAL) == 4) {
+            if (use_narrow3 && res_hdr_ok && !n3_nt && !(opts && (opts->variant_flags & 0x200000u))) {
+                uint32_t max_hops = 0;
+                for (uint32_t p = 0; p < nb_.n_packs; ++p) max_hops = std::max(max_hops, L.res.pack_hdr[8 * (size_t)p + 5] & 0xFFFFu);
+                onchip_hc = max_hops <= 10 ? 10 : max_hops <= 16 ? 16 : 0;
+                const uint32_t part = opts ? (opts->variant_flags >> 22) & 3u : 0u;
+                if (onchip_hc == 16) onchip_mode = 3;
+                if (part == 1 || part == 2) {
+                    if (onchip_hc == 10 && wpb == 4) onchip_mode = part;
+                    else onchip_hc = 0;
+                }
+                pot_on_chip = onchip_hc != 0;
+            }
+        }
         if (wb_.n_packs) {
             wide_threads = std::min<uint32_t>(1024, std::max<uint32_t>(64, ((wide_pack_width + 1) / 2 + 63) / 64 * 64));
             wide_npt = (wide_pack_width + wide_threads - 1) / wide_threads;
@@ -631,6 +647,7 @@
         Kern<WideFn> wide;
         Kern<MixedFn> mixed;
         HugeFn huge = nullptr;
+        bool reads_pot = true, stores_pot = true;
         const void* narrow_fn() const { return res2 ? (const void*)res2 : res ? (const void*)res : rec ? (const void*)rec : (const void*)narrow; }
     };
     struct Kernels {
@@ -642,6 +659,7 @@
         Kern<SmallFn> small;
         Kern<TransFn> transpose[2];
         Kern<LincombFn> lincomb[2];
+        Sweep onchip[2];
     } kern;
     Sweep ov_sweep[2];
     template <int MODE, bool OV>
@@ -699,12 +717,34 @@
         }
         return s;
     }
+    RecFn onchip_fn(bool bwd, bool rebuild, bool store) const
+    {
+        if (onchip_hc == 16) return pick<4, 8>(wpb, [&](auto W) -> RecFn { return &k_bwd_narrow4<REAL, W.value, 16, true, true>; });
+        if (rebuild && !store)
+            return pick<4, 8>(wpb, [&](auto W) -> RecFn {
+                return bwd ? &k_bwd_narrow4<REAL, W.value, 10, true, false> : &k_fwd_narrow4<REAL, W.value, 10, true, false>;
+            });
+        if (rebuild) return bwd ? &k_bwd_narrow4<REAL, 4, 10, true, true> : &k_fwd_narrow4<REAL, 4, 10, true, true>;
+        return bwd ? &k_bwd_narrow4<REAL, 4, 10, false, false> : &k_fwd_narrow4<REAL, 4, 10, false, false>;
+    }
     void resolve_kernels()
     {
         for (int bwd = 0; bwd < 2; ++bwd) {
             kern.sweep[bwd][FWD_PLAIN] = resolve_sweep<FWD_PLAIN, false>(bwd);
             kern.sweep[bwd][FWD_SOLVE] = resolve_sweep<FWD_SOLVE, false>(bwd);
             kern.sweep[bwd][FWD_SOLUTION] = resolve_sweep<FWD_SOLUTION, false>(bwd);
+        }
+        if (onchip_hc) {
+            for (int bwd = 0; bwd < 2; ++bwd) {
+                Sweep s = kern.sweep[bwd][FWD_SOLVE];
+                if (onchip_mode == 3 && !bwd) { kern.onchip[0] = s; continue; }
+                const bool rebuild = onchip_mode == 0 || (onchip_mode == 1) == !bwd;
+                const bool store = onchip_mode != 0 && rebuild;
+                if constexpr (sizeof(REAL) == 4) s.rec = onchip_fn(bwd, rebuild, onchip_mode == 3 || store);
+                s.reads_pot = !rebuild;
+                s.stores_pot = onchip_mode == 3 || store;
+                kern.onchip[bwd] = s;
+            }
         }
         kern.ex_threads = exch_small ? EXS_THREADS : exch_medium ? EXM_THREADS : EX_THREADS;
         pick<EXS_THREADS, EXM_THREADS, EX_THREADS>(kern.ex_threads, [&](auto T_) {
@@ -754,6 +794,9 @@
         for (const auto& dir : k.sweep)
             for (const Sweep& s : dir)
                 if ((rc = raise_lds_limits(s))) return rc;
+        if (onchip_hc)
+            for (const Sweep& s : k.onchip)
+                if ((rc = raise_lds_limits(s))) return rc;
         for (const auto* e : {&k.ex[0], &k.ex[1], &k.ex_w, &k.ex_raw})
             if ((rc = raise_lds_limit(*e))) return rc;
         for (const auto* e : {&k.seg[0], &k.seg[1], &k.seg_w})
@@ -872,12 +915,13 @@
         HIPCHK(hipSetDevice(device));
         int rc = launch_bwd(BWD_PLAIN, nullptr, REAL(0), BDDMMA_K_OTHER);
         if (rc) return rc;
-        bwd_valid = true;
-        return BDDMMA_OK;
-    }
+        bwd_valid = lb_valid = true;
+        return BDDMMA_OK;
+    }
+    int bound_run() { return lb_valid ? BDDMMA_OK : backward_run(); }
     int lower_bound(double* lb) override
     {
-        int rc = backward_run();
+        int rc = bound_run();
         if (rc) return rc;
         if (lb_cached) {
             *lb = lb_cache;
@@ -915,7 +959,7 @@
     int lower_bound_enqueue(int slot) override
     {
         if (slot < 0 || slot > 1) { err = "lower_bound_enqueue: slot must be 0 or 1"; return BDDMMA_ERR_INVALID_ARGUMENT; }
-        int rc = backward_run();
+        int rc = bound_run();
         if (rc) return rc;
         lb_slot_gen[slot] = lb_gen;
         if (lb_cached) {
@@ -939,7 +983,7 @@
             lb_slot_known[slot] = true;
         }
         *lb = lb_slot_value[slot];
-        if (lb_slot_gen[slot] == lb_gen && bwd_valid) {
+        if (lb_slot_gen[slot] == lb_gen && lb_valid) {
             lb_cache = *lb;
             lb_cached = true;
         }
@@ -962,28 +1006,32 @@
         return BDDMMA_OK;
     }
 
-    int mma_forward(REAL omega, const REAL* delta_lay, bool ov = false)
+    bool onchip_usable(bool ov) const { return onchip_hc != 0 && !ov && d_x_layer == nullptr; }
+    int mma_forward(REAL omega, const REAL* delta_lay, bool ov = false, bool on_chip = false)
     {
         int rc;
-        if (!bwd_valid && (rc = backward_run())) return rc;
-        rc = launch_sweep(false, ov ? ov_sweep[0] : kern.sweep[0][FWD_SOLVE], delta_lay, omega, BDDMMA_K_FORWARD_MM, ov);
+        const Sweep& s = ov ? ov_sweep[0] : (on_chip && onchip_usable(ov)) ? kern.onchip[0] : kern.sweep[0][FWD_SOLVE];
+        if (s.reads_pot && !bwd_valid && (rc = backward_run())) return rc;
+        rc = launch_sweep(false, s, delta_lay, omega, BDDMMA_K_FORWARD_MM, ov);
         x_layer_valid = false;
         if (rc) return rc;
-        fwd_valid = true;
-        bwd_valid = false;
-        return BDDMMA_OK;
-    }
-    int mma_backward(REAL omega, const REAL* delta_lay, bool ov = false)
-    {
-        if (!fwd_valid) {
+        fwd_valid = s.stores_pot;
+        bwd_valid = lb_valid = false;
+        return BDDMMA_OK;
+    }
+    int mma_backward(REAL omega, const REAL* delta_lay, bool ov = false, bool on_chip = false)
+    {
+        const Sweep& s = ov ? ov_sweep[1] : (on_chip && onchip_usable(ov)) ? kern.onchip[1] : kern.sweep[1][BWD_SOLVE];
+        if (s.reads_pot && !fwd_valid) {
             err = "backward_mm requires a valid forward state (call forward_mm first)";
             return BDDMMA_ERR_STATE;
         }
-        int rc = launch_sweep(true, ov ? ov_sweep[1] : kern.sweep[1][BWD_SOLVE], delta_lay, omega, BDDMMA_K_BACKWARD_MM, ov);
+        int rc = launch_sweep(true, s, delta_lay, omega, BDDMMA_K_BACKWARD_MM, ov);
         if (rc) return rc;
         x_layer_valid = d_x_layer != nullptr;
         fwd_valid = false;
-        bwd_valid = true;
+        bwd_valid = s.stores_pot;
+        lb_valid = true;
         return BDDMMA_OK;
     }
     bool small_usable() const { return small_ok && !profiling && d_x_layer == nullptr; }
@@ -993,7 +1041,7 @@
         ++lb_gen;
         x_layer_valid = false;
         fwd_valid = false;
-        bwd_valid = true;
+        bwd_valid = lb_valid = true;
         delta_var_valid = false;
     }
     int launch_small(REAL omega, uint32_t n, const RunStep& rstep)
@@ -1053,9 +1101,9 @@
         int rc;
         if (small_usable() && !run_stop) return launch_small((REAL)omega, 1, RunStep{});
         prof_active = profiling && (prof_iter++ % prof_stride == 0);
-        if ((rc = mma_forward((REAL)omega, d_delta_lay))) return rc;
+        if ((rc = mma_forward((REAL)omega, d_delta_lay, false, true))) return rc;
         if ((rc = exchange())) return rc;
-        if ((rc = mma_backward((REAL)omega, d_delta_lay))) return rc;
+        if ((rc = mma_backward((REAL)omega, d_delta_lay, false, true))) return rc;
         if ((rc = exchange(true))) return rc;
         return BDDMMA_OK;
     }
@@ -1536,7 +1584,7 @@
         int rc;
         if ((rc = forward_run())) return rc;
         if ((rc = launch_bwd(BWD_MARGINALS, nullptr, REAL(0), BDDMMA_K_OTHER))) return rc;
-        bwd_valid = true;
+        bwd_valid = lb_valid = true;
         return marginals_out(sorted, var, mm0, mm1, on_device);
     }
     int marginals_out(int sorted, int32_t* var, void* mm0, void* mm1, int on_device)
@@ -1651,7 +1699,7 @@
         int rc;
         if ((rc = forward_run())) return rc;
         if ((rc = launch_bwd(BWD_MARGINALS, nullptr, REAL(0), BDDMMA_K_OTHER))) return rc;
-        bwd_valid = true;
+        bwd_valid = lb_valid = true;
         REAL* dst = on_device ? (REAL*)out : d_tmp0;
         hipLaunchKernelGGL((k_diff<REAL, REAL>), dim3(cdiv(n_layers, 256)), dim3(256), 0, stream, dst, (const REAL*)d_tmp1, (const REAL*)d_tmp0, (uint32_t)n_layers);
         if (!on_device) return copy_out(out, dst, n_layers * sizeof(REAL), 0);
@@ -1844,7 +1892,7 @@
         if ((rc = distribute_delta())) return rc;
         if ((rc = forward_run())) return rc;
         if ((rc = launch_bwd(BWD_MARGINALS, nullptr, REAL(0), BDDMMA_K_OTHER))) return rc;
-        bwd_valid = true;
+        bwd_valid = lb_valid = true;
         HIPCHK(hipMemsetAsync(d_counts, 0, 4 * sizeof(uint32_t), stream));
         REAL* c0 = d_delta_c;
         REAL* c1 = d_delta_c + n_vars;
diff --git a/bdd_amd/csrc/solver_sm.hpp b/bdd_amd/csrc/solver_sm.hpp
--- a/bdd_amd/csrc/solver_sm.hpp
+++ b/bdd_amd/csrc/solver_sm.hpp
@@ -134,7 +134,7 @@
 template <typename REAL>
 int SolverT<REAL>::sm_launch_bwd()
 {
-    bwd_valid = false;
+    bwd_valid = lb_valid = false;
     lb_cached = false;
     ++lb_gen;
     return launch_pull(sm_bwd_sweep());
diff --git a/bdd_amd/solver.py b/bdd_amd/solver.py
--- a/bdd_amd/solver.py
+++ b/bdd_amd/solver.py
@@ -81,6 +81,9 @@
 
     def nontemporal_loads(self) -> bool:
         return bool(self._L.bddmma_nontemporal_loads(self._h))
+
+    def potentials_on_chip(self) -> bool:
+        return bool(self._L.bddmma_potentials_on_chip(self._h))
     def device(self) -> int:
         return int(self._L.bddmma_device(self._h))
     def device_bytes(self): return int(self._L.bddmma_device_bytes(self._h))
diff --git a/include/bdd_mma.h b/include/bdd_mma.h
--- a/include/bdd_mma.h
+++ b/include/bdd_mma.h
@@ -76,6 +76,7 @@
 int bddmma_fused_small(const bddmma_solver* s);
 int bddmma_fused_small_learned(const bddmma_solver* s);
 int bddmma_nontemporal_loads(const bddmma_solver* s);
+int bddmma_potentials_on_chip(const bddmma_solver* s);
 int bddmma_precision(const bddmma_solver* s);
 int bddmma_device(const bddmma_solver* s);
 int bddmma_num_bdds_per_var(const bddmma_solver* s, int32_t* out);
```

Measured after the change: 9529, median of 6. +8.6%, better.
